# olegiy/manuscript-ocr

Hardware: AMD Instinct MI355X
Metric: manuscript pages/sec end-to-end (EAST+TRBA) at 1/2/4/8 MI355X; CER vs CPU ref (higher is better)
Workload: dtype f32 (bf16x3 split operands on the 1x1 / Winograd-domain GEMMs, f32 accumulate)

## Files before the change

include/msocr.h:

```cpp
#ifndef MSOCR_H
#define MSOCR_H
#include <stdint.h>

#ifdef __cplusplus
extern "C" {
#endif

#define MSOCR_F32 0
#define MSOCR_BF16 1

#define MSOCR_OK 0
#define MSOCR_E_ARG (-1)
#define MSOCR_E_LAUNCH (-2)
#define MSOCR_E_NOGPU (-3)

#define MSOCR_CONV_RELU 1u
#define MSOCR_CONV_RESIDUAL 2u
#define MSOCR_CONV_POOL2 4u

typedef struct msocr_conv_desc {
  int32_t dtype;
  int32_t N, H, W, Cin;
  int64_t in_sN, in_sH, in_sW;
  int32_t KH, KW, stride_h, stride_w, pad_h, pad_w;
  int32_t Ho, Wo, Cout;
  int64_t out_ld;
  int64_t res_ld;
  uint32_t flags;
} msocr_conv_desc;

int msocr_conv2d(const msocr_conv_desc* d, const void* in, const void* weight, const float* bias,
                 const void* residual, void* out, void* stream);

#define MSOCR_WINO_2X2 0
#define MSOCR_WINO_4X2 1
#define MSOCR_WINO_4X4 2
int64_t msocr_winograd_workspace_bytes(const msocr_conv_desc* d, int form);
int msocr_winograd_weights_host(int form, const float* w_khwc_host, int Cout, int Cin, float* u_out_host);
int msocr_conv3x3_winograd(const msocr_conv_desc* d, int form, int split, const void* in, const void* u, const float* bias,
                           const void* residual, void* out, void* workspace, void* stream);
int msocr_winograd_input_transform(const msocr_conv_desc* d, int form, const void* in, void* workspace, void* stream);
int msocr_winograd_gemm(const msocr_conv_desc* d, int form, int split, const void* u, void* workspace, void* stream);
int msocr_winograd_output_transform(const msocr_conv_desc* d, int form, const void* workspace, const float* bias, const void* residual,
                                    void* out, void* stream);

int msocr_split_bf16x3_host(const float* w_host, int64_t n, uint16_t* planes_out_host);
int msocr_split_bf16x3_ktile_host(const float* w_host, int64_t nbatch, int64_t rows, int64_t k, uint16_t* planes_out_host);
int msocr_conv1x1_split(const msocr_conv_desc* d, const void* in, const void* weight_planes, const float* bias,
                        const void* residual, void* out, void* stream);
int msocr_conv2d_split(const msocr_conv_desc* d, const void* in, const void* weight_planes, const float* bias,
                       const void* residual, void* out, void* stream);

int64_t msocr_winograd_fused64_workspace_bytes(const msocr_conv_desc* d);
int msocr_conv3x3_winograd_fused64(const msocr_conv_desc* d, int split, const void* in, const void* u, const float* bias,
                                   const void* residual, void* out, void* workspace, void* stream);
int msocr_winograd_fused64_gemm_output(const msocr_conv_desc* d, int split, const void* u, const void* workspace, const float* bias,
                                       const void* residual, void* out, void* stream);

int msocr_normalize_u8(const uint8_t* src, int N, int H, int W, int pad_t, int pad_l, int Hp, int Wp, int cpad,
                       int mode, int dtype, void* out, void* stream);

int msocr_resize_linear_u8(const uint8_t* src, int N, int sh, int sw, uint8_t* dst, int dh, int dw, void* stream);

int msocr_maxpool2d(const void* in, int N, int H, int W, int C, int64_t in_ld, int k, int s, int p, int dtype,
                    void* out, int Ho, int Wo, int64_t out_ld, void* stream);

int msocr_upsample2x_bilinear(const void* in, int N, int H, int W, int C, int64_t in_ld, int dtype, void* out,
                              int64_t out_ld, void* stream);

int msocr_east_head(const void* h1, int64_t npix, int64_t in_ld, int dtype, const float* w9, const float* b9,
                    float* score_out, float* geo_out, void* stream);

int msocr_east_decode(const float* score, const float* geo, int N, int H, int W, float thresh, float scale,
                      int quant, float* cand_out, int32_t* count_out, int max_cand, void* stream);

int64_t msocr_lanms_workspace_bytes(int N, int max_cand);
int msocr_east_lanms(const float* cand, const int32_t* counts, int N, int max_cand, double iou_thr, float* boxes_out,
                     int32_t* nbox_out, void* workspace, void* stream);

int64_t msocr_east_box_tail_workspace_bytes(int N, int max_cand);
int msocr_east_box_tail(const float* boxes, const int32_t* nbox, int N, int max_cand, double expand_w, double expand_h,
                        double scale_x, double scale_y, int axis_aligned_output, int remove_anomalies, double sigma, int min_count,
                        float* out, int32_t* n_out, void* workspace, void* stream);
int msocr_east_box_tail_host(const float* quads_host, int M, double expand_w, double expand_h, double scale_x, double scale_y,
                             int axis_aligned_output, int remove_anomalies, double sigma, int min_count, float* out_host,
                             int32_t* n_out_host);


int msocr_se_residual(const void* x, const void* identity, int N, int HW, int C, int dtype, const float* w1,
                      const float* w2, float* gate_ws, void* out, void* stream);

int msocr_mean_over_h(const void* in, int N, int H, int W, int C, int dtype, float* out, void* stream);

int msocr_bilstm_recurrent(const float* xproj, const float* w_hh_t, int B, int T, int H, float* hcat_out,
                           void* stream);
int msocr_bilstm_recurrent_split(const float* xproj, const uint16_t* whh_planes, int B, int T, int H, float* hcat_out,
                                 void* stream);

typedef struct msocr_attn_weights {
  const float* h2h_wt;
  const float* h2h_b;
  const float* score_w;
  const float* wih_ctx_t;
  const float* wih_tok;
  const float* whh_t;
  const float* b_gates;
  const float* gen_wt;
  const float* gen_b;
} msocr_attn_weights;

int msocr_attn_greedy(const float* batch_H, const float* proj_H, const msocr_attn_weights* w, int B, int T, int H,
                      int V, int steps, int sos_id, int eos_id, int blank_id, float* logits_out, int32_t* ids_out,
                      void* stream);
int64_t msocr_attn_beam_workspace_bytes(int B, int steps, int beam, int V);
int msocr_attn_beam(const float* batch_H, const float* proj_H, const msocr_attn_weights* w, int B, int T, int H,
                    int V, int steps, int beam, const float* lp_dev, float temperature, int sos_id, int eos_id,
                    int blank_id, int32_t* fin_step_out, void* workspace, const int32_t* chunk_id_dev,
                    const int32_t* chunk_size_dev, int32_t* chunk_state_dev, void* stream);
typedef struct msocr_attn_split_weights {
  const uint16_t* h2h_p;
  const uint16_t* whh_p;
  const uint16_t* gen_p;
} msocr_attn_split_weights;

int msocr_attn_beam_hoisted(const float* batch_H, const float* proj_H, const float* ctx_gates, const msocr_attn_weights* w,
                            const msocr_attn_split_weights* ws, int B, int T, int H, int V, int steps, int beam, const float* lp_dev,
                            float temperature, int sos_id, int eos_id, int blank_id, int32_t* fin_step_out, void* workspace,
                            const int32_t* chunk_id_dev, const int32_t* chunk_size_dev, int32_t* chunk_state_dev, void* stream);
int msocr_attn_greedy_hoisted(const float* batch_H, const float* proj_H, const float* ctx_gates, const msocr_attn_weights* w,
                              const msocr_attn_split_weights* ws, int B, int T, int H, int V, int steps, int sos_id, int eos_id,
                              int blank_id, float* logits_out, int32_t* ids_out, void* stream);
int64_t msocr_attn_pack_split_elems(int N);
int msocr_attn_pack_split_host(const float* wt_host, int N, int gate_interleaved, uint16_t* out_host);
int msocr_attn_beam_finalize(const void* workspace, int B, int V, int steps, int beam, const int32_t* trun_dev,
                             float* logits_out, int32_t* ids_out, void* stream);

int msocr_seq_confidence(const float* logits, const int32_t* ids, const int32_t* trun_dev, int B, int V, int steps,
                         float* conf_out, void* stream);

int msocr_crop_resize_pad(const uint8_t* pages, int N, int H, int W, const int32_t* desc_dev,
                          const int32_t* desc_host, int M, int img_h, int img_w, uint8_t* canvases, void* stream);

int msocr_reading_order_host(const int32_t* boxes_host, int n, double y_tol_ratio, double x_gap_ratio,
                             int32_t* order_out_host);

int64_t msocr_reading_order_workspace_bytes(int N, int max_cand);
int msocr_reading_order_crops(const float* boxes, const int32_t* nbox, int N, int max_cand, int page_h, int page_w,
                              int min_text_size, int img_h, int img_w, double y_tol_ratio, double x_gap_ratio, int page_base,
                              int32_t* order_out, int32_t* keep_out, int32_t* desc_out, int32_t* ncrop_out, void* workspace,
                              void* stream);

typedef struct msocr_jpeg_info {
  int32_t width, height, ncomp;
  int32_t hs[3], vs[3];
  int32_t blocks_w[3], blocks_h[3];
  int32_t supported;
  int64_t coef_off[3];
  int64_t coef_total;
  uint16_t quant[3][64];
} msocr_jpeg_info;
int msocr_jpeg_parse_host(const uint8_t* data_host, int64_t len, msocr_jpeg_info* info_out);
int msocr_jpeg_entropy_decode_host(const uint8_t* data_host, int64_t len, const msocr_jpeg_info* info, int16_t* coef_out_host);
int64_t msocr_jpeg_scan_desc_bytes(void);
int64_t msocr_jpeg_scan_prepare_host(const uint8_t* data_host, int64_t len, const msocr_jpeg_info* info, int64_t bytes_base,
                                     void* desc_out, uint32_t* bounds_out, int64_t bounds_cap);
int msocr_jpeg_entropy_decode_device(const uint8_t* bytes_dev, const void* descs_dev, int32_t n_pages, int32_t max_intervals,
                                     const uint32_t* bounds_dev, const int64_t* page_base_dev, int16_t* coef_dev, int64_t coef_total,
                                     int32_t* status_dev, void* stream);
int msocr_jpeg_entropy_decode_intervals_host(const uint8_t* bytes_host, const void* descs_host, int32_t n_pages,
                                             const uint32_t* bounds_host, const int64_t* page_base_host, int16_t* coef_host,
                                             int64_t coef_total, int32_t* status_host);
int64_t msocr_jpeg_workspace_bytes(const msocr_jpeg_info* info);
int msocr_jpeg_reconstruct(const msocr_jpeg_info* info, const int16_t* coef_dev, void* workspace_dev, uint8_t* rgb_out_dev,
                           void* stream);
int msocr_jpeg_reconstruct_host(const msocr_jpeg_info* info, const int16_t* coef_host, uint8_t* rgb_out_host);

int msocr_nchw_f32_to_nhwc(const float* in, int N, int C, int H, int W, int dtype, void* out, int64_t out_ld,
                           void* stream);
int msocr_nhwc_to_nchw_f32(const void* in, int N, int C, int H, int W, int64_t in_ld, int dtype, float* out,
                           void* stream);

const char* msocr_version(void);

#ifdef __cplusplus
}
#endif
#endif
```

manuscript_ocr_amd/_native.py:

```python
import ctypes
import os

import torch

_HERE = os.path.dirname(os.path.abspath(__file__))
LIB_PATH = os.path.join(_HERE, "libmsocr.so")

F32, BF16 = 0, 1
CONV_RELU, CONV_RESIDUAL, CONV_POOL2 = 1, 2, 4
WINO_2X2, WINO_4X2, WINO_4X4 = 0, 1, 2

c_i32, c_i64, c_u32 = ctypes.c_int32, ctypes.c_int64, ctypes.c_uint32
c_f32, c_f64, c_vp = ctypes.c_float, ctypes.c_double, ctypes.c_void_p


class ConvDesc(ctypes.Structure):
    _fields_ = [
        ("dtype", c_i32), ("N", c_i32), ("H", c_i32), ("W", c_i32), ("Cin", c_i32),
        ("in_sN", c_i64), ("in_sH", c_i64), ("in_sW", c_i64),
        ("KH", c_i32), ("KW", c_i32), ("stride_h", c_i32), ("stride_w", c_i32), ("pad_h", c_i32), ("pad_w", c_i32),
        ("Ho", c_i32), ("Wo", c_i32), ("Cout", c_i32),
        ("out_ld", c_i64), ("res_ld", c_i64), ("flags", c_u32),
    ]


class JpegInfo(ctypes.Structure):
    _fields_ = [("width", c_i32), ("height", c_i32), ("ncomp", c_i32), ("hs", c_i32 * 3), ("vs", c_i32 * 3),
                ("blocks_w", c_i32 * 3), ("blocks_h", c_i32 * 3), ("supported", c_i32), ("coef_off", c_i64 * 3),
                ("coef_total", c_i64), ("quant", (ctypes.c_uint16 * 64) * 3)]


class AttnWeights(ctypes.Structure):
    _fields_ = [(n, c_vp) for n in ("h2h_wt", "h2h_b", "score_w", "wih_ctx_t", "wih_tok", "whh_t", "b_gates", "gen_wt", "gen_b")]


class AttnSplitWeights(ctypes.Structure):
    _fields_ = [(n, c_vp) for n in ("h2h_p", "whh_p", "gen_p")]


_SIGS = {
    "msocr_conv2d": (c_i32, [ctypes.POINTER(ConvDesc), c_vp, c_vp, c_vp, c_vp, c_vp, c_vp]),
    "msocr_winograd_workspace_bytes": (c_i64, [ctypes.POINTER(ConvDesc), c_i32]),
    "msocr_winograd_weights_host": (c_i32, [c_i32, c_vp, c_i32, c_i32, c_vp]),
    "msocr_conv3x3_winograd": (c_i32, [ctypes.POINTER(ConvDesc), c_i32, c_i32, c_vp, c_vp, c_vp, c_vp, c_vp, c_vp, c_vp]),
    "msocr_winograd_input_transform": (c_i32, [ctypes.POINTER(ConvDesc), c_i32, c_vp, c_vp, c_vp]),
    "msocr_winograd_gemm": (c_i32, [ctypes.POINTER(ConvDesc), c_i32, c_i32, c_vp, c_vp, c_vp]),
    "msocr_winograd_output_transform": (c_i32, [ctypes.POINTER(ConvDesc), c_i32, c_vp, c_vp, c_vp, c_vp, c_vp]),
    "msocr_winograd_fused64_workspace_bytes": (c_i64, [ctypes.POINTER(ConvDesc)]),
    "msocr_conv3x3_winograd_fused64": (c_i32, [ctypes.POINTER(ConvDesc), c_i32, c_vp, c_vp, c_vp, c_vp, c_vp, c_vp, c_vp]),
    "msocr_winograd_fused64_gemm_output": (c_i32, [ctypes.POINTER(ConvDesc), c_i32, c_vp, c_vp, c_vp, c_vp, c_vp, c_vp]),
    "msocr_split_bf16x3_host": (c_i32, [c_vp, c_i64, c_vp]),
    "msocr_split_bf16x3_ktile_host": (c_i32, [c_vp, c_i64, c_i64, c_i64, c_vp]),
    "msocr_conv1x1_split": (c_i32, [ctypes.POINTER(ConvDesc), c_vp, c_vp, c_vp, c_vp, c_vp, c_vp]),
    "msocr_conv2d_split": (c_i32, [ctypes.POINTER(ConvDesc), c_vp, c_vp, c_vp, c_vp, c_vp, c_vp]),
    "msocr_normalize_u8": (c_i32, [c_vp, c_i32, c_i32, c_i32, c_i32, c_i32, c_i32, c_i32, c_i32, c_i32, c_i32, c_vp, c_vp]),
    "msocr_resize_linear_u8": (c_i32, [c_vp, c_i32, c_i32, c_i32, c_vp, c_i32, c_i32, c_vp]),
    "msocr_maxpool2d": (c_i32, [c_vp, c_i32, c_i32, c_i32, c_i32, c_i64, c_i32, c_i32, c_i32, c_i32, c_vp, c_i32, c_i32, c_i64, c_vp]),
    "msocr_upsample2x_bilinear": (c_i32, [c_vp, c_i32, c_i32, c_i32, c_i32, c_i64, c_i32, c_vp, c_i64, c_vp]),
    "msocr_east_head": (c_i32, [c_vp, c_i64, c_i64, c_i32, c_vp, c_vp, c_vp, c_vp, c_vp]),
    "msocr_east_decode": (c_i32, [c_vp, c_vp, c_i32, c_i32, c_i32, c_f32, c_f32, c_i32, c_vp, c_vp, c_i32, c_vp]),
    "msocr_lanms_workspace_bytes": (c_i64, [c_i32, c_i32]),
    "msocr_east_lanms": (c_i32, [c_vp, c_vp, c_i32, c_i32, c_f64, c_vp, c_vp, c_vp, c_vp]),
    "msocr_se_residual": (c_i32, [c_vp, c_vp, c_i32, c_i32, c_i32, c_i32, c_vp, c_vp, c_vp, c_vp, c_vp]),
    "msocr_mean_over_h": (c_i32, [c_vp, c_i32, c_i32, c_i32, c_i32, c_i32, c_vp, c_vp]),
    "msocr_bilstm_recurrent": (c_i32, [c_vp, c_vp, c_i32, c_i32, c_i32, c_vp, c_vp]),
    "msocr_bilstm_recurrent_split": (c_i32, [c_vp, c_vp, c_i32, c_i32, c_i32, c_vp, c_vp]),
    "msocr_attn_greedy": (c_i32, [c_vp, c_vp, ctypes.POINTER(AttnWeights), c_i32, c_i32, c_i32, c_i32, c_i32, c_i32, c_i32, c_i32,
                                  c_vp, c_vp, c_vp]),
    "msocr_attn_greedy_hoisted": (c_i32, [c_vp, c_vp, c_vp, ctypes.POINTER(AttnWeights), ctypes.POINTER(AttnSplitWeights), c_i32, c_i32,
                                          c_i32, c_i32, c_i32, c_i32, c_i32, c_i32, c_vp, c_vp, c_vp]),
    "msocr_attn_beam": (c_i32, [c_vp, c_vp, ctypes.POINTER(AttnWeights), c_i32, c_i32, c_i32, c_i32, c_i32, c_i32, c_vp, c_f32,
                                c_i32, c_i32, c_i32, c_vp, c_vp, c_vp, c_vp, c_vp, c_vp]),
    "msocr_attn_pack_split_elems": (c_i64, [c_i32]),
    "msocr_attn_pack_split_host": (c_i32, [c_vp, c_i32, c_i32, c_vp]),
    "msocr_attn_beam_hoisted": (c_i32, [c_vp, c_vp, c_vp, ctypes.POINTER(AttnWeights), ctypes.POINTER(AttnSplitWeights), c_i32, c_i32, c_i32, c_i32, c_i32, c_i32, c_vp, c_f32,
                                        c_i32, c_i32, c_i32, c_vp, c_vp, c_vp, c_vp, c_vp, c_vp]),
    "msocr_attn_beam_workspace_bytes": (c_i64, [c_i32, c_i32, c_i32, c_i32]),
    "msocr_attn_beam_finalize": (c_i32, [c_vp, c_i32, c_i32, c_i32, c_i32, c_vp, c_vp, c_vp, c_vp]),
    "msocr_seq_confidence": (c_i32, [c_vp, c_vp, c_vp, c_i32, c_i32, c_i32, c_vp, c_vp]),
    "msocr_crop_resize_pad": (c_i32, [c_vp, c_i32, c_i32, c_i32, c_vp, c_vp, c_i32, c_i32, c_i32, c_vp, c_vp]),
    "msocr_east_box_tail_workspace_bytes": (c_i64, [c_i32, c_i32]),
    "msocr_east_box_tail": (c_i32, [c_vp, c_vp, c_i32, c_i32, c_f64, c_f64, c_f64, c_f64, c_i32, c_i32, c_f64, c_i32, c_vp, c_vp, c_vp, c_vp]),
    "msocr_east_box_tail_host": (c_i32, [c_vp, c_i32, c_f64, c_f64, c_f64, c_f64, c_i32, c_i32, c_f64, c_i32, c_vp, c_vp]),
    "msocr_reading_order_host": (c_i32, [c_vp, c_i32, c_f64, c_f64, c_vp]),
    "msocr_reading_order_workspace_bytes": (c_i64, [c_i32, c_i32]),
    "msocr_reading_order_crops": (c_i32, [c_vp, c_vp, c_i32, c_i32, c_i32, c_i32, c_i32, c_i32, c_i32, c_f64, c_f64, c_i32,
                                          c_vp, c_vp, c_vp, c_vp, c_vp, c_vp]),
    "msocr_jpeg_parse_host": (c_i32, [c_vp, c_i64, ctypes.POINTER(JpegInfo)]),
    "msocr_jpeg_entropy_decode_host": (c_i32, [c_vp, c_i64, ctypes.POINTER(JpegInfo), c_vp]),
    "msocr_jpeg_scan_desc_bytes": (c_i64, []),
    "msocr_jpeg_scan_prepare_host": (c_i64, [c_vp, c_i64, ctypes.POINTER(JpegInfo), c_i64, c_vp, c_vp, c_i64]),
    "msocr_jpeg_entropy_decode_device": (c_i32, [c_vp, c_vp, c_i32, c_i32, c_vp, c_vp, c_vp, c_i64, c_vp, c_vp]),
    "msocr_jpeg_entropy_decode_intervals_host": (c_i32, [c_vp, c_vp, c_i32, c_vp, c_vp, c_vp, c_i64, c_vp]),
    "msocr_jpeg_workspace_bytes": (c_i64, [ctypes.POINTER(JpegInfo)]),
    "msocr_jpeg_reconstruct": (c_i32, [ctypes.POINTER(JpegInfo), c_vp, c_vp, c_vp, c_vp]),
    "msocr_jpeg_reconstruct_host": (c_i32, [ctypes.POINTER(JpegInfo), c_vp, c_vp]),
    "msocr_nchw_f32_to_nhwc": (c_i32, [c_vp, c_i32, c_i32, c_i32, c_i32, c_i32, c_vp, c_i64, c_vp]),
    "msocr_nhwc_to_nchw_f32": (c_i32, [c_vp, c_i32, c_i32, c_i32, c_i32, c_i64, c_i32, c_vp, c_vp]),
    "msocr_version": (ctypes.c_char_p, []),
}

_lib = None


class NativeError(RuntimeError):
    pass


def lib():
    global _lib
    if _lib is None:
        if not os.path.exists(LIB_PATH) and os.path.exists("/opt/rocm/bin/hipcc"):
            import fcntl
            import subprocess
            try:
                with open(os.path.join(_HERE, "csrc", ".build.lock"), "w") as lock:
                    fcntl.flock(lock, fcntl.LOCK_EX)
                    if not os.path.exists(LIB_PATH):
                        subprocess.check_call(["make", "-s", "-j4", "-C", os.path.join(_HERE, "csrc"), "ARCH=gfx950"])
            except Exception as e:
                print(f"[manuscript_ocr_amd] building libmsocr.so failed: {e}")
        if not os.path.exists(LIB_PATH):
            raise NativeError(
                f"{LIB_PATH} not found: build it with `python -c 'import __graft_entry__ as g; g.build()'` "
                "(or `make -C manuscript_ocr_amd/csrc`). There is no CPU fallback."
            )
        L = ctypes.CDLL(LIB_PATH)
        missing = [name for name in _SIGS if not hasattr(L, name)]
        if missing:
            raise NativeError(f"{LIB_PATH} lacks symbols declared in include/msocr.h: {missing}")
        for name, (res, args) in _SIGS.items():
            fn = getattr(L, name)
            fn.restype, fn.argtypes = res, args
        _lib = L
    return _lib


def exported_symbols():
    return list(_SIGS)


def check(rc, what):
    if rc != 0:
        raise NativeError(f"{what} failed with code {rc} (-1 bad argument/shape, -2 launch failure)")
```

manuscript_ocr_amd/csrc/trba_kernels.hip:

```cpp
#include <hip/hip_runtime.h>
#include <math.h>
#include <stdint.h>

#include "internal.h"
#include "msocr.h"

#define MSOCR_LAUNCH(...) do { (void)hipGetLastError(); hipLaunchKernelGGL(__VA_ARGS__); } while (0)
#define LAUNCH_OK() (hipGetLastError() == hipSuccess ? MSOCR_OK : MSOCR_E_LAUNCH)

typedef float f32x4 __attribute__((ext_vector_type(4)));

__device__ __forceinline__ float bf2f(uint16_t v) { return __uint_as_float(((uint32_t)v) << 16); }
__device__ __forceinline__ uint16_t f2bf(float f) {
  __bf16 b = (__bf16)f;
  return *reinterpret_cast<uint16_t*>(&b);
}
template <typename T> __device__ __forceinline__ float ldf(const T* p);
template <> __device__ __forceinline__ float ldf<float>(const float* p) { return *p; }
template <> __device__ __forceinline__ float ldf<uint16_t>(const uint16_t* p) { return bf2f(*p); }
template <typename T> __device__ __forceinline__ void stf(T* p, float v);
template <> __device__ __forceinline__ void stf<float>(float* p, float v) { *p = v; }
template <> __device__ __forceinline__ void stf<uint16_t>(uint16_t* p, float v) { *p = f2bf(v); }

__device__ __forceinline__ float sigmoidf_(float x) { return 1.0f / (1.0f + expf(-x)); }

__device__ __forceinline__ float wave_sum(float v) {
#pragma unroll
  for (int o = 32; o > 0; o >>= 1) v += __shfl_xor(v, o);
  return v;
}

template <typename T>
__device__ __forceinline__ f32x4 ld4(const T* p);
template <>
__device__ __forceinline__ f32x4 ld4<float>(const float* p) { return *reinterpret_cast<const f32x4*>(p); }
template <>
__device__ __forceinline__ f32x4 ld4<uint16_t>(const uint16_t* p) {
  const uint2 v = *reinterpret_cast<const uint2*>(p);
  f32x4 r = {bf2f((uint16_t)(v.x & 0xffff)), bf2f((uint16_t)(v.x >> 16)), bf2f((uint16_t)(v.y & 0xffff)), bf2f((uint16_t)(v.y >> 16))};
  return r;
}
template <typename T>
__device__ __forceinline__ void st4(T* p, f32x4 v);
template <>
__device__ __forceinline__ void st4<float>(float* p, f32x4 v) { *reinterpret_cast<f32x4*>(p) = v; }
template <>
__device__ __forceinline__ void st4<uint16_t>(uint16_t* p, f32x4 v) {
  uint2 o;
  o.x = (uint32_t)f2bf(v[0]) | ((uint32_t)f2bf(v[1]) << 16);
  o.y = (uint32_t)f2bf(v[2]) | ((uint32_t)f2bf(v[3]) << 16);
  *reinterpret_cast<uint2*>(p) = o;
}

template <typename T, int NT>
__global__ __launch_bounds__(NT) void se_residual_kernel(const T* __restrict__ x, const T* __restrict__ idt, int HW, int C,
                                                           const float* __restrict__ w1, const float* __restrict__ w2,
                                                           float* __restrict__ gate_ws, T* __restrict__ out) {
  extern __shared__ __attribute__((aligned(16))) float sm[];
  const int n = blockIdx.x, tid = threadIdx.x;
  const int C4 = C / 4, PG = NT / C4;
  float* part = sm;
  float* mean = sm + PG * C;
  float* hid = mean + C;
  float* gate = hid + C / 16;
  const T* xs = x + (long)n * HW * C;
  const int cg = tid % C4, pg = tid / C4;
  {
    f32x4 s = {0.f, 0.f, 0.f, 0.f};
    int p = pg;
    for (; p + 3 * PG < HW; p += 4 * PG) {
      f32x4 v[4];
#pragma unroll
      for (int u = 0; u < 4; ++u) v[u] = ld4<T>(xs + (long)(p + u * PG) * C + cg * 4);
#pragma unroll
      for (int u = 0; u < 4; ++u) { s[0] += v[u][0]; s[1] += v[u][1]; s[2] += v[u][2]; s[3] += v[u][3]; }
    }
    for (; p < HW; p += PG) {
      const f32x4 v = ld4<T>(xs + (long)p * C + cg * 4);
      s[0] += v[0]; s[1] += v[1]; s[2] += v[2]; s[3] += v[3];
    }
    *reinterpret_cast<f32x4*>(&part[pg * C + cg * 4]) = s;
  }
  __syncthreads();
  const float inv = 1.0f / (float)HW;
  for (int c = tid; c < C; c += NT) {
    float s = 0.f;
    for (int g = 0; g < PG; ++g) s += part[g * C + c];
    mean[c] = s * inv;
  }
  __syncthreads();
  const int Cr = C / 16;
  {
    const int lane = tid & 63, wv = tid >> 6;
    for (int j = wv; j < Cr; j += NT / 64) {
      float a = 0.f;
      for (int c = lane; c < C; c += 64) a = fmaf(w1[(long)j * C + c], mean[c], a);
      a = wave_sum(a);
      if (lane == 0) hid[j] = fmaxf(a, 0.f);
    }
  }
  __syncthreads();
  for (int c = tid; c < C; c += NT) {
    float a = 0.f;
    for (int j = 0; j < Cr; ++j) a = fmaf(w2[(long)c * Cr + j], hid[j], a);
    const float g = sigmoidf_(a);
    gate[c] = g;
    gate_ws[(long)n * C + c] = g;
  }
  __syncthreads();
  const T* is = idt + (long)n * HW * C;
  T* os = out + (long)n * HW * C;
  const f32x4 g4 = *reinterpret_cast<const f32x4*>(&gate[cg * 4]);
  int p = pg;
  for (; p + 3 * PG < HW; p += 4 * PG) {
    f32x4 v[4], r[4];
#pragma unroll
    for (int u = 0; u < 4; ++u) {
      const long o = (long)(p + u * PG) * C + cg * 4;
      v[u] = ld4<T>(xs + o);
      r[u] = ld4<T>(is + o);
    }
#pragma unroll
    for (int u = 0; u < 4; ++u) {
      f32x4 y;
#pragma unroll
      for (int e = 0; e < 4; ++e) y[e] = fmaxf(v[u][e] * g4[e] + r[u][e], 0.f);
      st4<T>(os + (long)(p + u * PG) * C + cg * 4, y);
    }
  }
  for (; p < HW; p += PG) {
    const long o = (long)p * C + cg * 4;
    const f32x4 v = ld4<T>(xs + o), r = ld4<T>(is + o);
    f32x4 y;
#pragma unroll
    for (int e = 0; e < 4; ++e) y[e] = fmaxf(v[e] * g4[e] + r[e], 0.f);
    st4<T>(os + o, y);
  }
}

extern "C" int msocr_se_residual(const void* x, const void* identity, int N, int HW, int C, int dtype, const float* w1, const float* w2,
                                 float* gate_ws, void* out, void* stream) {
  if (!x || !identity || !w1 || !w2 || !gate_ws || !out || N <= 0 || HW <= 0 || C < 64 || C > 1024 || (C & (C - 1))) return MSOCR_E_ARG;
  hipStream_t s = (hipStream_t)stream;
  if (dtype == MSOCR_F32) {
    MSOCR_LAUNCH((se_residual_kernel<float, 1024>), dim3(N), dim3(1024), (size_t)((1024 / (C / 4)) * C + 2 * C + C / 16) * sizeof(float), s,
                 (const float*)x, (const float*)identity, HW, C, w1, w2, gate_ws, (float*)out);
  } else if (dtype == MSOCR_BF16) {
    MSOCR_LAUNCH((se_residual_kernel<uint16_t, 256>), dim3(N), dim3(256), (size_t)((1024 / C) * C + 2 * C + C / 16) * sizeof(float), s,
                 (const uint16_t*)x, (const uint16_t*)identity, HW, C, w1, w2, gate_ws, (uint16_t*)out);
  } else {
    return MSOCR_E_ARG;
  }
  return LAUNCH_OK();
}

template <typename T>
__global__ void mean_over_h_kernel(const T* __restrict__ in, int N, int H, int W, int C, float* __restrict__ out) {
  const long total = (long)N * W * C;
  for (long i = blockIdx.x * (long)blockDim.x + threadIdx.x; i < total; i += (long)gridDim.x * blockDim.x) {
    const int c = (int)(i % C);
    const long t = i / C;
    const int w = (int)(t % W);
    const int n = (int)(t / W);
    float s = 0.f;
    for (int h = 0; h < H; ++h) s += ldf<T>(in + (((long)n * H + h) * W + w) * C + c);
    out[i] = s / (float)H;
  }
}
extern "C" int msocr_mean_over_h(const void* in, int N, int H, int W, int C, int dtype, float* out, void* stream) {
  if (!in || !out || N <= 0 || H <= 0 || W <= 0 || C <= 0) return MSOCR_E_ARG;
  const long total = (long)N * W * C;
  long g = (total + 255) / 256;
  if (g > 2048) g = 2048;
  hipStream_t s = (hipStream_t)stream;
  if (dtype == MSOCR_F32)
    MSOCR_LAUNCH(mean_over_h_kernel<float>, dim3((unsigned)g), dim3(256), 0, s, (const float*)in, N, H, W, C, out);
  else if (dtype == MSOCR_BF16)
    MSOCR_LAUNCH(mean_over_h_kernel<uint16_t>, dim3((unsigned)g), dim3(256), 0, s, (const uint16_t*)in, N, H, W, C, out);
  else
    return MSOCR_E_ARG;
  return LAUNCH_OK();
}

#define LSTM_RB 4
template <int H>
__global__ __launch_bounds__(H) void bilstm_kernel(const float* __restrict__ xproj, const float* __restrict__ whh_t, int B, int T,
                                                    float* __restrict__ hcat) {
  constexpr int G = 4 * H, RB = LSTM_RB;
  __shared__ __attribute__((aligned(16))) float hs[2][H][RB];
  const int j = threadIdx.x, d = blockIdx.y;
  const int b0 = blockIdx.x * RB;
  const float* wt = whh_t + (long)d * H * G;
  float c[RB];
#pragma unroll
  for (int r = 0; r < RB; ++r) {
    c[r] = 0.f;
    hs[0][j][r] = 0.f;
  }
  __syncthreads();
  for (int s = 0; s < T; ++s) {
    const int t = d == 0 ? s : T - 1 - s;
    const int cur = s & 1;
    float acc[4][RB];
#pragma unroll
    for (int r = 0; r < RB; ++r) {
      const int b = b0 + r < B ? b0 + r : B - 1;
      const float* xp = xproj + (((long)b * T + t) * 2 + d) * G;
#pragma unroll
      for (int g = 0; g < 4; ++g) acc[g][r] = xp[g * H + j];
    }
#pragma unroll 1
    for (int k0 = 0; k0 < H; k0 += 8) {
      f32x4 wq[8];
#pragma unroll
      for (int u = 0; u < 8; ++u) wq[u] = *reinterpret_cast<const f32x4*>(&wt[((long)(k0 + u) * H + j) * 4]);
#pragma unroll
      for (int u = 0; u < 8; ++u) {
        float hv[RB];
#pragma unroll
        for (int r4 = 0; r4 < RB; r4 += 4) {
          const f32x4 hq = *reinterpret_cast<const f32x4*>(&hs[cur][k0 + u][r4]);
          hv[r4] = hq[0]; hv[r4 + 1] = hq[1]; hv[r4 + 2] = hq[2]; hv[r4 + 3] = hq[3];
        }
#pragma unroll
        for (int g = 0; g < 4; ++g) {
#pragma unroll
          for (int r = 0; r < RB; ++r) acc[g][r] = fmaf(wq[u][g], hv[r], acc[g][r]);
        }
      }
    }
#pragma unroll
    for (int r = 0; r < RB; ++r) {
      const float ig = sigmoidf_(acc[0][r]), fg = sigmoidf_(acc[1][r]), gg = tanhf(acc[2][r]), og = sigmoidf_(acc[3][r]);
      c[r] = fg * c[r] + ig * gg;
      const float h = og * tanhf(c[r]);
      hs[cur ^ 1][j][r] = h;
      if (b0 + r < B) hcat[((long)(b0 + r) * T + t) * (2 * H) + d * H + j] = h;
    }
    __syncthreads();
  }
}

extern "C" int msocr_bilstm_recurrent(const float* xproj, const float* w_hh_t, int B, int T, int H, float* hcat_out, void* stream) {
  if (!xproj || !w_hh_t || !hcat_out || B <= 0 || T <= 0) return MSOCR_E_ARG;
  const dim3 grid((B + LSTM_RB - 1) / LSTM_RB, 2);
  if (H == 256) MSOCR_LAUNCH(bilstm_kernel<256>, grid, dim3(256), 0, (hipStream_t)stream, xproj, w_hh_t, B, T, hcat_out);
  else if (H == 128) MSOCR_LAUNCH(bilstm_kernel<128>, grid, dim3(128), 0, (hipStream_t)stream, xproj, w_hh_t, B, T, hcat_out);
  else if (H == 512) MSOCR_LAUNCH(bilstm_kernel<512>, grid, dim3(512), 0, (hipStream_t)stream, xproj, w_hh_t, B, T, hcat_out);
  else if (H == 64) MSOCR_LAUNCH(bilstm_kernel<64>, grid, dim3(64), 0, (hipStream_t)stream, xproj, w_hh_t, B, T, hcat_out);
  else if (H == 192) MSOCR_LAUNCH(bilstm_kernel<192>, grid, dim3(192), 0, (hipStream_t)stream, xproj, w_hh_t, B, T, hcat_out);
  else if (H == 320) MSOCR_LAUNCH(bilstm_kernel<320>, grid, dim3(320), 0, (hipStream_t)stream, xproj, w_hh_t, B, T, hcat_out);
  else if (H == 384) MSOCR_LAUNCH(bilstm_kernel<384>, grid, dim3(384), 0, (hipStream_t)stream, xproj, w_hh_t, B, T, hcat_out);
  else if (H == 448) MSOCR_LAUNCH(bilstm_kernel<448>, grid, dim3(448), 0, (hipStream_t)stream, xproj, w_hh_t, B, T, hcat_out);
  else return MSOCR_E_ARG;
  return LAUNCH_OK();
}


__global__ void attn_beam_finalize_kernel(const float* __restrict__ ws_logits, const int32_t* __restrict__ back,
                                          const int32_t* __restrict__ tokv, const int32_t* __restrict__ best_at,
                                          const int32_t* __restrict__ trun, int V, int steps, int K, float* __restrict__ logits_out,
                                          int32_t* __restrict__ ids_out) {
  const int b = blockIdx.x, tid = threadIdx.x;
  __shared__ int path[64];
  const int tr = trun[b];
  if (tid == 0) {
    int cur = best_at[(long)b * steps + tr - 1];
    for (int t = tr - 1; t >= 0; --t) {
      const long o = ((long)b * steps + t) * K + cur;
      ids_out[(long)b * steps + t] = tokv[o];
      path[t] = back[o];
      cur = back[o];
    }
    for (int t = tr; t < steps; ++t) ids_out[(long)b * steps + t] = -1;
  }
  __syncthreads();
  for (int t = 0; t < tr; ++t)
    for (int v = tid; v < V; v += blockDim.x)
      logits_out[((long)b * steps + t) * V + v] = ws_logits[(((long)b * steps + t) * K + path[t]) * V + v];
}

static bool attn_mfma_shape(int T, int H, int V) { return H == 256 && V <= 256 && T <= 48; }
static int check_attn(const float* bh, const float* ph, const msocr_attn_weights* w, int B, int T, int H, int V, int steps) {
  if (!bh || !ph || !w || B <= 0 || T <= 0 || T > 64 || H < 64 || H > 512 || H % 64 || V <= 0 || V > 512 || steps <= 0 || steps > 64)
    return MSOCR_E_ARG;
  if (!w->h2h_wt || !w->h2h_b || !w->score_w || !w->wih_ctx_t || !w->wih_tok || !w->whh_t || !w->b_gates || !w->gen_wt || !w->gen_b)
    return MSOCR_E_ARG;
  return MSOCR_OK;
}

extern "C" int msocr_attn_greedy(const float* batch_H, const float* proj_H, const msocr_attn_weights* w, int B, int T, int H, int V,
                                 int steps, int sos_id, int eos_id, int blank_id, float* logits_out, int32_t* ids_out, void* stream) {
  if (check_attn(batch_H, proj_H, w, B, T, H, V, steps) || !logits_out || !ids_out) return MSOCR_E_ARG;
  if (sos_id < 0 || sos_id >= V) return MSOCR_E_ARG;
  AttnArgs a{};
  a.batch_H = batch_H; a.proj_H = proj_H; a.w = *w;
  a.B = B; a.T = T; a.V = V; a.steps = steps; a.K = 1;
  a.sos_id = sos_id; a.eos_id = eos_id; a.blank_id = blank_id; a.temperature = 1.0f;
  a.logits_out = logits_out; a.ids_out = ids_out;
  return msocr_internal_attn_general(a, H, false, (hipStream_t)stream);
}

extern "C" int msocr_attn_greedy_hoisted(const float* batch_H, const float* proj_H, const float* ctx_gates, const msocr_attn_weights* w,
                                         const msocr_attn_split_weights* ws, int B, int T, int H, int V, int steps, int sos_id, int eos_id,
                                         int blank_id, float* logits_out, int32_t* ids_out, void* stream) {
  if (check_attn(batch_H, proj_H, w, B, T, H, V, steps) || !logits_out || !ids_out) return MSOCR_E_ARG;
  if (sos_id < 0 || sos_id >= V || !attn_mfma_shape(T, H, V)) return MSOCR_E_ARG;
  if (!ctx_gates || ((uintptr_t)ctx_gates & 15)) return MSOCR_E_ARG;
  if (!ws || !ws->h2h_p || !ws->whh_p || !ws->gen_p || (((uintptr_t)ws->h2h_p | (uintptr_t)ws->whh_p | (uintptr_t)ws->gen_p) & 15))
    return MSOCR_E_ARG;
  AttnArgs a{};
  a.batch_H = batch_H; a.proj_H = proj_H; a.w = *w; a.ctx_gates = ctx_gates;
  a.h2h_p = ws->h2h_p; a.whh_p = ws->whh_p; a.gen_p = ws->gen_p;
  a.B = B; a.T = T; a.V = V; a.steps = steps; a.K = 1;
  a.sos_id = sos_id; a.eos_id = eos_id; a.blank_id = blank_id; a.temperature = 1.0f;
  a.logits_out = logits_out; a.ids_out = ids_out;
  return msocr_internal_attn_greedy_mfma(a, (hipStream_t)stream);
}

static inline int64_t beam_ws_logits(int B, int steps, int K, int V) { return (int64_t)B * steps * K * V * 4; }
extern "C" int64_t msocr_attn_beam_workspace_bytes(int B, int steps, int beam, int V) {
  if (B <= 0 || steps <= 0 || beam <= 0 || V <= 0) return 0;
  return beam_ws_logits(B, steps, beam, V) + (int64_t)B * steps * beam * 8 + (int64_t)B * steps * 4 + 256;
}

static int attn_beam_impl(const float* batch_H, const float* proj_H, const float* ctx_gates, const msocr_attn_weights* w,
                          const msocr_attn_split_weights* ws, int B, int T, int H, int V, int steps, int beam, const float* lp_dev, float temperature, int sos_id, int eos_id, int blank_id,
                          int32_t* fin_step_out, void* workspace, const int32_t* chunk_id_dev, const int32_t* chunk_size_dev,
                          int32_t* chunk_state_dev, void* stream) {
  if (check_attn(batch_H, proj_H, w, B, T, H, V, steps) || !fin_step_out || !workspace) return MSOCR_E_ARG;
  if (beam < 1 || beam > 16 || sos_id < 0 || sos_id >= V || ((uintptr_t)workspace & 15)) return MSOCR_E_ARG;
  if (ctx_gates && (!attn_mfma_shape(T, H, V) || beam > 8)) return MSOCR_E_ARG;
  AttnArgs a{};
  a.batch_H = batch_H; a.proj_H = proj_H; a.w = *w; a.ctx_gates = ctx_gates;
  if (ws) { a.h2h_p = ws->h2h_p; a.whh_p = ws->whh_p; a.gen_p = ws->gen_p; }
  a.B = B; a.T = T; a.V = V; a.steps = steps; a.K = beam;
  a.sos_id = sos_id; a.eos_id = eos_id; a.blank_id = blank_id; a.temperature = temperature; a.lp = lp_dev;
  char* p = (char*)workspace;
  a.logits_out = (float*)p; p += beam_ws_logits(B, steps, beam, V);
  a.back = (int32_t*)p; p += (int64_t)B * steps * beam * 4;
  a.tokv = (int32_t*)p; p += (int64_t)B * steps * beam * 4;
  a.best_at = (int32_t*)p;
  a.fin_step = fin_step_out;
  if (chunk_id_dev && chunk_size_dev && chunk_state_dev) { a.chunk_id = chunk_id_dev; a.chunk_size = chunk_size_dev; a.chunk_state = chunk_state_dev; }
  if (!ctx_gates) return msocr_internal_attn_general(a, H, true, (hipStream_t)stream);
  return msocr_internal_attn_beam_mfma(a, (hipStream_t)stream);
}

extern "C" int msocr_attn_beam(const float* batch_H, const float* proj_H, const msocr_attn_weights* w, int B, int T, int H, int V,
                               int steps, int beam, const float* lp_dev, float temperature, int sos_id, int eos_id, int blank_id,
                               int32_t* fin_step_out, void* workspace, const int32_t* chunk_id_dev, const int32_t* chunk_size_dev,
                               int32_t* chunk_state_dev, void* stream) {
  return attn_beam_impl(batch_H, proj_H, nullptr, w, nullptr, B, T, H, V, steps, beam, lp_dev, temperature, sos_id, eos_id, blank_id, fin_step_out,
                        workspace, chunk_id_dev, chunk_size_dev, chunk_state_dev, stream);
}

extern "C" int msocr_attn_beam_hoisted(const float* batch_H, const float* proj_H, const float* ctx_gates, const msocr_attn_weights* w,
                                       const msocr_attn_split_weights* ws, int B, int T, int H, int V, int steps, int beam,
                                       const float* lp_dev, float temperature, int sos_id, int eos_id, int blank_id, int32_t* fin_step_out,
                                       void* workspace, const int32_t* chunk_id_dev, const int32_t* chunk_size_dev,
                                       int32_t* chunk_state_dev, void* stream) {
  if (!ctx_gates || ((uintptr_t)ctx_gates & 15)) return MSOCR_E_ARG;
  if (ws && (!ws->h2h_p || !ws->whh_p || !ws->gen_p || (((uintptr_t)ws->h2h_p | (uintptr_t)ws->whh_p | (uintptr_t)ws->gen_p) & 15)))
    return MSOCR_E_ARG;
  return attn_beam_impl(batch_H, proj_H, ctx_gates, w, ws, B, T, H, V, steps, beam, lp_dev, temperature, sos_id, eos_id, blank_id,
                        fin_step_out, workspace, chunk_id_dev, chunk_size_dev, chunk_state_dev, stream);
}

extern "C" int msocr_attn_beam_finalize(const void* workspace, int B, int V, int steps, int beam, const int32_t* trun_dev,
                                        float* logits_out, int32_t* ids_out, void* stream) {
  if (!workspace || !trun_dev || !logits_out || !ids_out || B <= 0 || V <= 0 || steps <= 0 || steps > 64 || beam < 1 || beam > 16)
    return MSOCR_E_ARG;
  const char* p = (const char*)workspace;
  const float* wl = (const float*)p; p += beam_ws_logits(B, steps, beam, V);
  const int32_t* back = (const int32_t*)p; p += (int64_t)B * steps * beam * 4;
  const int32_t* tokv = (const int32_t*)p; p += (int64_t)B * steps * beam * 4;
  const int32_t* best_at = (const int32_t*)p;
  MSOCR_LAUNCH(attn_beam_finalize_kernel, dim3(B), dim3(256), 0, (hipStream_t)stream, wl, back, tokv, best_at, trun_dev, V, steps, beam,
               logits_out, ids_out);
  return LAUNCH_OK();
}

__global__ __launch_bounds__(64) void seq_confidence_kernel(const float* __restrict__ logits, const int32_t* __restrict__ ids,
                                                             const int32_t* __restrict__ trun, int V, int steps,
                                                             float* __restrict__ conf) {
  const int b = blockIdx.x, lane = threadIdx.x;
  const int tr = trun[b];
  float acc = 0.f;
  for (int t = 0; t < tr; ++t) {
    const float* x = logits + ((long)b * steps + t) * V;
    float m = -INFINITY;
    for (int v = lane; v < V; v += 64) m = fmaxf(m, x[v]);
#pragma unroll
    for (int o = 32; o > 0; o >>= 1) m = fmaxf(m, __shfl_xor(m, o));
    float s = 0.f;
    for (int v = lane; v < V; v += 64) s += expf(x[v] - m);
    s = wave_sum(s);
    const int id = ids[(long)b * steps + t];
    const float logp = (x[id] - m) - logf(s);
    acc += expf(logp);
  }
  if (lane == 0) conf[b] = tr > 0 ? acc / (float)tr : 0.f;
}

extern "C" int msocr_seq_confidence(const float* logits, const int32_t* ids, const int32_t* trun_dev, int B, int V, int steps,
                                    float* conf_out, void* stream) {
  if (!logits || !ids || !trun_dev || !conf_out || B <= 0 || V <= 0 || steps <= 0) return MSOCR_E_ARG;
  MSOCR_LAUNCH(seq_confidence_kernel, dim3(B), dim3(64), 0, (hipStream_t)stream, logits, ids, trun_dev, V, steps, conf_out);
  return LAUNCH_OK();
}
```

manuscript_ocr_amd/csrc/winograd.hip:

```cpp
#include <hip/hip_runtime.h>
#include <stdint.h>

#include "internal.h"
#include "msocr.h"

#define MSOCR_LAUNCH(...) do { (void)hipGetLastError(); hipLaunchKernelGGL(__VA_ARGS__); } while (0)

typedef float f32x4 __attribute__((ext_vector_type(4)));

template <int M> __device__ void wino_bt1(const f32x4 d[M + 2], f32x4 r[M + 2]);
template <int M> __device__ void wino_at1(const f32x4 m[M + 2], f32x4 y[M]);

template <> __device__ __forceinline__ void wino_bt1<2>(const f32x4 d[4], f32x4 r[4]) {
  r[0] = d[0] - d[2];
  r[1] = d[1] + d[2];
  r[2] = d[2] - d[1];
  r[3] = d[1] - d[3];
}
template <> __device__ __forceinline__ void wino_at1<2>(const f32x4 m[4], f32x4 y[2]) {
  y[0] = (m[0] + m[1]) + m[2];
  y[1] = (m[1] - m[2]) - m[3];
}

__device__ __forceinline__ void wino44_bt(const f32x4 d[6], f32x4 r[6]) {
  constexpr float k97_36 = 97.0f / 36.0f, k4_9 = 4.0f / 9.0f, k9_4 = 2.25f, k3_2 = 1.5f, k2_3 = 2.0f / 3.0f;
#pragma unroll
  for (int e = 0; e < 4; ++e) {
    r[0][e] = fmaf(-k97_36, d[2][e], d[0][e]) + d[4][e];
    r[5][e] = fmaf(-k97_36, d[3][e], d[1][e]) + d[5][e];
    const float e1 = fmaf(-k4_9, d[2][e], d[4][e]), o1 = fmaf(k3_2, d[3][e], -k2_3 * d[1][e]);
    const float e2 = fmaf(-k9_4, d[2][e], d[4][e]), o2 = fmaf(k2_3, d[3][e], -k3_2 * d[1][e]);
    r[1][e] = e1 + o1; r[2][e] = e1 - o1;
    r[3][e] = e2 + o2; r[4][e] = e2 - o2;
  }
}
__device__ __forceinline__ void wino44_at(const f32x4 m[6], f32x4 y[4]) {
  constexpr float k3_2 = 1.5f, k2_3 = 2.0f / 3.0f, k9_4 = 2.25f, k4_9 = 4.0f / 9.0f, k27_8 = 3.375f, k8_27 = 8.0f / 27.0f;
#pragma unroll
  for (int e = 0; e < 4; ++e) {
    const float p12 = m[1][e] + m[2][e], d12 = m[1][e] - m[2][e], p34 = m[3][e] + m[4][e], d34 = m[3][e] - m[4][e];
    y[0][e] = (m[0][e] + p12) + p34;
    y[1][e] = fmaf(k3_2, d12, k2_3 * d34);
    y[2][e] = fmaf(k9_4, p12, k4_9 * p34);
    y[3][e] = fmaf(k27_8, d12, k8_27 * d34) + m[5][e];
  }
}
template <> __device__ __forceinline__ void wino_bt1<4>(const f32x4 d[6], f32x4 r[6]) { wino44_bt(d, r); }
template <> __device__ __forceinline__ void wino_at1<4>(const f32x4 m[6], f32x4 y[4]) { wino44_at(m, y); }


struct WinoGeom {
  int N, H, W;
  int TH, TW;
  long Mt;
};

template <int MH, int MW>
__device__ __forceinline__ void wino_input_body(const float* in, long sN, long sH, long sW, int C, WinoGeom g, float* V) {
  constexpr int PH = MH + 2, PW = MW + 2;
  constexpr bool w_first = MH == 4;
  const int cch = C >> 2;
  const long gid = (long)blockIdx.x * 256 + threadIdx.x;
  const long t = gid / cch;
  const int c = (int)(gid - t * cch) << 2;
  if (t >= g.Mt) return;
  const int tw = (int)(t % g.TW);
  const long r = t / g.TW;
  const int th = (int)(r % g.TH);
  const int n = (int)(r / g.TH);
  const int h0 = MH * th - 1, w0 = MW * tw - 1;
  const float* base = in + (long)n * sN + c;
  f32x4 q[PH][PW];
#pragma unroll
  for (int i = 0; i < PH; ++i) {
    const int hi = h0 + i;
    const bool okh = (unsigned)hi < (unsigned)g.H;
    f32x4 d[PW];
#pragma unroll
    for (int j = 0; j < PW; ++j) {
      const int wi = w0 + j;
      const bool ok = okh && (unsigned)wi < (unsigned)g.W;
      const f32x4 v = *reinterpret_cast<const f32x4*>(ok ? base + (long)hi * sH + (long)wi * sW : base);
      d[j] = ok ? v : (f32x4){0.f, 0.f, 0.f, 0.f};
    }
    if constexpr (w_first) {
      wino_bt1<MW>(d, q[i]);
    } else {
#pragma unroll
      for (int j = 0; j < PW; ++j) q[i][j] = d[j];
    }
  }
  const long plane = g.Mt * (long)C;
  float* o = V + t * (long)C + c;
  if constexpr (w_first) {
#pragma unroll
    for (int j = 0; j < PW; ++j) {
      f32x4 col[PH], v[PH];
#pragma unroll
      for (int i = 0; i < PH; ++i) col[i] = q[i][j];
      wino_bt1<MH>(col, v);
#pragma unroll
      for (int i = 0; i < PH; ++i) *reinterpret_cast<f32x4*>(o + (i * PW + j) * plane) = v[i];
    }
  } else {
#pragma unroll
    for (int i = 0; i < PH; ++i) {
      f32x4 row[PW], v[PW];
#pragma unroll
      for (int j = 0; j < PW; ++j) {
        f32x4 col[PH], hv[PH];
#pragma unroll
        for (int k = 0; k < PH; ++k) col[k] = q[k][j];
        wino_bt1<MH>(col, hv);
        row[j] = hv[i];
      }
      wino_bt1<MW>(row, v);
#pragma unroll
      for (int j = 0; j < PW; ++j) *reinterpret_cast<f32x4*>(o + (i * PW + j) * plane) = v[j];
    }
  }
}

template <int MH, int MW>
__device__ __forceinline__ void wino_output_body(const float* Mw, int Cout, WinoGeom g, const float* bias, const float* res, long res_ld,
                                                 int relu, float* out, long out_ld) {
  constexpr int PH = MH + 2, PW = MW + 2;
  const int cch = Cout >> 2;
  const long gid = (long)blockIdx.x * 256 + threadIdx.x;
  const long t = gid / cch;
  const int c = (int)(gid - t * cch) << 2;
  if (t >= g.Mt) return;
  const int tw = (int)(t % g.TW);
  const long r = t / g.TW;
  const int th = (int)(r % g.TH);
  const int n = (int)(r / g.TH);
  const long plane = g.Mt * (long)Cout;
  const float* mp = Mw + t * (long)Cout + c;
  f32x4 mt[PH][PW];
  if constexpr (MH == 2) {
#pragma unroll
    for (int i = 0; i < PH; ++i)
#pragma unroll
      for (int j = 0; j < PW; ++j) mt[i][j] = *reinterpret_cast<const f32x4*>(mp + (i * PW + j) * plane);
  }
  f32x4 s[MH][PW];
#pragma unroll
  for (int j = 0; j < PW; ++j) {
    f32x4 m[PH], y[MH];
#pragma unroll
    for (int i = 0; i < PH; ++i) m[i] = MH == 2 ? mt[i][j] : *reinterpret_cast<const f32x4*>(mp + (i * PW + j) * plane);
    wino_at1<MH>(m, y);
#pragma unroll
    for (int a = 0; a < MH; ++a) s[a][j] = y[a];
  }
  f32x4 b = {0.f, 0.f, 0.f, 0.f};
  if (bias) b = *reinterpret_cast<const f32x4*>(bias + c);
#pragma unroll
  for (int a = 0; a < MH; ++a) {
    const int ho = MH * th + a;
    if (ho >= g.H) continue;
    f32x4 y[MW];
    wino_at1<MW>(s[a], y);
#pragma unroll
    for (int j = 0; j < MW; ++j) {
      const int wo = MW * tw + j;
      if (wo >= g.W) continue;
      const long pix = ((long)n * g.H + ho) * g.W + wo;
      f32x4 v = y[j] + b;
      if (res) v += *reinterpret_cast<const f32x4*>(res + pix * res_ld + c);
      if (relu) {
        v[0] = fmaxf(v[0], 0.f); v[1] = fmaxf(v[1], 0.f); v[2] = fmaxf(v[2], 0.f); v[3] = fmaxf(v[3], 0.f);
      }
      *reinterpret_cast<f32x4*>(out + pix * out_ld + c) = v;
    }
  }
}

#define WINO_TRANSFORM_KERNELS(PREFIX, MH, MW)                                                                                    \
  __global__ __launch_bounds__(256) void PREFIX##_input_kernel(const float* __restrict__ in, long sN, long sH, long sW, int C,   \
                                                               WinoGeom g, float* __restrict__ V) {                            \
    wino_input_body<MH, MW>(in, sN, sH, sW, C, g, V);                                                                            \
  }                                                                                                                              \
  __global__ __launch_bounds__(256) void PREFIX##_output_kernel(const float* __restrict__ Mw, int Cout, WinoGeom g,              \
                                                                const float* __restrict__ bias, const float* __restrict__ res,  \
                                                                long res_ld, int relu, float* __restrict__ out, long out_ld) {  \
    wino_output_body<MH, MW>(Mw, Cout, g, bias, res, res_ld, relu, out, out_ld);                                                 \
  }
WINO_TRANSFORM_KERNELS(wino, 2, 2)
WINO_TRANSFORM_KERNELS(wino42, 4, 2)
WINO_TRANSFORM_KERNELS(wino44, 4, 4)
#undef WINO_TRANSFORM_KERNELS

static const int kWinoTile[3][2] = {{2, 2}, {4, 2}, {4, 4}};

static int wino_points(int form) { return (kWinoTile[form][0] + 2) * (kWinoTile[form][1] + 2); }

static bool wino_geom(const msocr_conv_desc* d, int form, WinoGeom* g) {
  if (form < MSOCR_WINO_2X2 || form > MSOCR_WINO_4X4 || !d || d->dtype != MSOCR_F32) return false;
  if (d->KH != 3 || d->KW != 3 || d->stride_h != 1 || d->stride_w != 1 || d->pad_h != 1 || d->pad_w != 1) return false;
  if (d->N <= 0 || d->H <= 0 || d->W <= 0 || d->Ho != d->H || d->Wo != d->W) return false;
  if (d->Cin <= 0 || d->Cin % 16 || d->Cout <= 0 || d->Cout % 32) return false;
  if ((long)d->N * ((d->H + 1) / 2) * ((d->W + 1) / 2) > 0x7fffffffL) return false;
  const int mh = kWinoTile[form][0], mw = kWinoTile[form][1];
  g->N = d->N; g->H = d->H; g->W = d->W;
  g->TH = (d->H + mh - 1) / mh; g->TW = (d->W + mw - 1) / mw;
  g->Mt = (long)d->N * g->TH * g->TW;
  return wino_points(form) * g->Mt * (long)(d->Cin > d->Cout ? d->Cin : d->Cout) <= 0x3fffffffffffL;
}

static bool wino_strides_ok(const msocr_conv_desc* d) { return !(d->in_sN % 4 || d->in_sH % 4 || d->in_sW % 4); }

static int wino_check(const msocr_conv_desc* d, int form, WinoGeom* g) {
  if (!wino_geom(d, form, g) || !wino_strides_ok(d) || d->out_ld % 4 || d->out_ld < d->Cout) return MSOCR_E_ARG;
  return MSOCR_OK;
}

static bool wino_gemm_ok(int form, int split) {
  if (split != 0 && split != 1) return false;
  return form == MSOCR_WINO_4X2 || (form == MSOCR_WINO_2X2 && !split) || (form == MSOCR_WINO_4X4 && split);
}

extern "C" int64_t msocr_winograd_workspace_bytes(const msocr_conv_desc* d, int form) {
  WinoGeom g;
  if (!wino_geom(d, form, &g)) return -1;
  return wino_points(form) * g.Mt * ((int64_t)d->Cin + d->Cout) * (int64_t)sizeof(float);
}

static int wino_launch_input(const msocr_conv_desc* d, int form, const WinoGeom& g, const void* in, void* workspace, void* stream) {
  if (!in || !workspace || (((uintptr_t)in | (uintptr_t)workspace) & 15)) return MSOCR_E_ARG;
  const long nb_in = (g.Mt * (d->Cin / 4) + 255) / 256;
  if (nb_in > 0x7fffffffL) return MSOCR_E_ARG;
  const dim3 grid((unsigned)nb_in), blk(256);
  hipStream_t st = (hipStream_t)stream;
  const float* x = (const float*)in;
  float* V = (float*)workspace;
  if (form == MSOCR_WINO_2X2) MSOCR_LAUNCH(wino_input_kernel, grid, blk, 0, st, x, (long)d->in_sN, (long)d->in_sH, (long)d->in_sW, d->Cin, g, V);
  else if (form == MSOCR_WINO_4X2) MSOCR_LAUNCH(wino42_input_kernel, grid, blk, 0, st, x, (long)d->in_sN, (long)d->in_sH, (long)d->in_sW, d->Cin, g, V);
  else MSOCR_LAUNCH(wino44_input_kernel, grid, blk, 0, st, x, (long)d->in_sN, (long)d->in_sH, (long)d->in_sW, d->Cin, g, V);
  return hipGetLastError() == hipSuccess ? MSOCR_OK : MSOCR_E_LAUNCH;
}

extern "C" int msocr_winograd_input_transform(const msocr_conv_desc* d, int form, const void* in, void* workspace, void* stream) {
  WinoGeom g;
  if (wino_check(d, form, &g) != MSOCR_OK) return MSOCR_E_ARG;
  return wino_launch_input(d, form, g, in, workspace, stream);
}

extern "C" int msocr_winograd_gemm(const msocr_conv_desc* d, int form, int split, const void* u, void* workspace, void* stream) {
  WinoGeom g;
  if (!wino_gemm_ok(form, split) || wino_check(d, form, &g) != MSOCR_OK || !u || !workspace) return MSOCR_E_ARG;
  if (split && (d->Cin % 32 || d->Cout % 64)) return MSOCR_E_ARG;
  const int P = wino_points(form);
  float* V = (float*)workspace;
  float* Mw = V + P * g.Mt * (long)d->Cin;
  if (split) return msocr_internal_gemm_split_batched(V, (const uint16_t*)u, Mw, g.Mt, d->Cout, d->Cin, P, (hipStream_t)stream);
  return msocr_internal_gemm_f32_batched(V, (const float*)u, Mw, g.Mt, d->Cout, d->Cin, P, (hipStream_t)stream);
}

extern "C" int msocr_winograd_output_transform(const msocr_conv_desc* d, int form, const void* workspace, const float* bias,
                                               const void* residual, void* out, void* stream) {
  WinoGeom g;
  if (wino_check(d, form, &g) != MSOCR_OK || !out || !workspace) return MSOCR_E_ARG;
  if (((uintptr_t)out | (uintptr_t)workspace) & 15) return MSOCR_E_ARG;
  const bool has_res = (d->flags & MSOCR_CONV_RESIDUAL) != 0;
  if (has_res && (!residual || d->res_ld % 4 || d->res_ld < d->Cout || ((uintptr_t)residual & 15))) return MSOCR_E_ARG;
  if (bias && ((uintptr_t)bias & 15)) return MSOCR_E_ARG;
  const long nb_out = (g.Mt * (d->Cout / 4) + 255) / 256;
  if (nb_out > 0x7fffffffL) return MSOCR_E_ARG;
  const float* Mw = (const float*)workspace + wino_points(form) * g.Mt * (long)d->Cin;
  const float* rp = has_res ? (const float*)residual : nullptr;
  const int relu = (d->flags & MSOCR_CONV_RELU) ? 1 : 0;
  const dim3 grid((unsigned)nb_out), blk(256);
  hipStream_t st = (hipStream_t)stream;
  float* o = (float*)out;
  if (form == MSOCR_WINO_2X2) MSOCR_LAUNCH(wino_output_kernel, grid, blk, 0, st, Mw, d->Cout, g, bias, rp, (long)d->res_ld, relu, o, (long)d->out_ld);
  else if (form == MSOCR_WINO_4X2) MSOCR_LAUNCH(wino42_output_kernel, grid, blk, 0, st, Mw, d->Cout, g, bias, rp, (long)d->res_ld, relu, o, (long)d->out_ld);
  else MSOCR_LAUNCH(wino44_output_kernel, grid, blk, 0, st, Mw, d->Cout, g, bias, rp, (long)d->res_ld, relu, o, (long)d->out_ld);
  return hipGetLastError() == hipSuccess ? MSOCR_OK : MSOCR_E_LAUNCH;
}

extern "C" int msocr_conv3x3_winograd(const msocr_conv_desc* d, int form, int split, const void* in, const void* u, const float* bias,
                                      const void* residual, void* out, void* workspace, void* stream) {
  if (!u || !wino_gemm_ok(form, split)) return MSOCR_E_ARG;
  int rc = msocr_winograd_input_transform(d, form, in, workspace, stream);
  if (rc != MSOCR_OK) return rc;
  rc = msocr_winograd_gemm(d, form, split, u, workspace, stream);
  if (rc != MSOCR_OK) return rc;
  return msocr_winograd_output_transform(d, form, workspace, bias, residual, out, stream);
}

typedef unsigned int u32x4w __attribute__((ext_vector_type(4)));
#ifndef WINO_FUSED_PFD
#define WINO_FUSED_PFD 3
#endif

typedef __bf16 bf16x8w __attribute__((ext_vector_type(8)));
typedef unsigned int u32x2w __attribute__((ext_vector_type(2)));
__device__ __forceinline__ unsigned int wino_split_step(float& x, float& y) {
  typedef __bf16 bf16x2 __attribute__((ext_vector_type(2)));
  typedef float f32x2 __attribute__((ext_vector_type(2)));
  const f32x2 v = {x, y};
  const bf16x2 h = __builtin_convertvector(v, bf16x2);
  const unsigned int pk = __builtin_bit_cast(unsigned int, h);
  x -= __uint_as_float(pk << 16);
  y -= __uint_as_float(pk & 0xffff0000u);
  return pk;
}

template <bool POOL, bool SPLIT = false>
__global__ __launch_bounds__(256, 3) void wino42_fused64_kernel(const float* __restrict__ V, const void* __restrict__ Uv, int Cout,
                                                                 WinoGeom g, const float* __restrict__ bias,
                                                                 const float* __restrict__ res, long res_ld, int relu,
                                                                 float* __restrict__ out, long out_ld) {
  constexpr int K = 64, BM = 32, BN = 32, ROWB = K * 4;
  constexpr int ROWS = 128, PLANE = BM * ROWS;
  constexpr int STAGE_BYTES = SPLIT ? 6 * PLANE : (BM + BN) * ROWB;
  __shared__ __attribute__((aligned(16))) unsigned char smem[2][STAGE_BYTES];
  const int tid = threadIdx.x, lane = tid & 63, wave = tid >> 6;
  const int mi = wave >> 1, nj = wave & 1;
  const int r16 = lane & 15, kg = lane >> 4;
  const int nbn = Cout / BN;
  const long nblk = (long)gridDim.x;
  long bid = blockIdx.x;
  {
    const long q = nblk >> 3, r = nblk & 7, x = bid & 7;
    bid = (x < r ? x * (q + 1) : r * (q + 1) + (x - r) * q) + (bid >> 3);
  }
  const int nb = (int)(bid % nbn);
  const long m0 = (bid / nbn) * BM;
  const int n0 = nb * BN;
  f32x4 acc[24];

  if constexpr (SPLIT) {
    const unsigned short* U = reinterpret_cast<const unsigned short*>(Uv);
    const int chunk = tid & 15, row0 = tid >> 4;
    const int bchunk = tid & 7, brow = tid >> 3;
    const long planeV = g.Mt * (long)K, planeU = (long)Cout * K, uplane = 24 * planeU;
    const float* pa[2];
#pragma unroll
    for (int i = 0; i < 2; ++i) {
      long m = m0 + row0 + 16 * i;
      if (m >= g.Mt) m = g.Mt - 1;
      pa[i] = V + m * K + chunk * 4;
    }
    const unsigned short* pb = U + (long)(n0 + brow) * K + bchunk * 8;
    constexpr int PFD = 2;
    u32x4w ra[PFD][2], rb[PFD][3];
    auto gload = [&](int p) {
#pragma unroll
      for (int i = 0; i < 2; ++i) ra[p % PFD][i] = *reinterpret_cast<const u32x4w*>(pa[i] + p * planeV);
#pragma unroll
      for (int pl = 0; pl < 3; ++pl) rb[p % PFD][pl] = *reinterpret_cast<const u32x4w*>(pb + pl * uplane + p * planeU);
    };
    auto sstore = [&](int p) {
      unsigned char* st = &smem[p & 1][0];
#pragma unroll
      for (int i = 0; i < 2; ++i) {
        const int row = row0 + 16 * i;
        float x0 = __uint_as_float(ra[p % PFD][i][0]), x1 = __uint_as_float(ra[p % PFD][i][1]);
        float x2 = __uint_as_float(ra[p % PFD][i][2]), x3 = __uint_as_float(ra[p % PFD][i][3]);
        unsigned char* dst = st + row * ROWS + (((chunk >> 1) ^ (row & 7)) << 4) + ((chunk & 1) << 3);
#pragma unroll
        for (int pl = 0; pl < 3; ++pl) {
          u32x2w v;
          v[0] = wino_split_step(x0, x1);
          v[1] = wino_split_step(x2, x3);
          *reinterpret_cast<u32x2w*>(dst + pl * PLANE) = v;
        }
      }
#pragma unroll
      for (int pl = 0; pl < 3; ++pl)
        *reinterpret_cast<u32x4w*>(st + (3 + pl) * PLANE + brow * ROWS + ((bchunk ^ (brow & 7)) << 4)) = rb[p % PFD][pl];
    };
#pragma unroll
    for (int q = 0; q < PFD; ++q) gload(q);
    sstore(0);
    __syncthreads();
#pragma unroll
    for (int p = 0; p < 24; ++p) {
      if (p + PFD < 24) gload(p + PFD);
      const unsigned char* st = &smem[p & 1][0];
      const int rowa = mi * 16 + r16, rowb = nj * 16 + r16;
      f32x4 c4 = {0.f, 0.f, 0.f, 0.f};
#pragma unroll
      for (int ks = 0; ks < 2; ++ks) {
        const int c = 4 * ks + kg;
        bf16x8w fa[3], fb[3];
#pragma unroll
        for (int pl = 0; pl < 3; ++pl) {
          fa[pl] = *reinterpret_cast<const bf16x8w*>(st + pl * PLANE + rowa * ROWS + ((c ^ (rowa & 7)) << 4));
          fb[pl] = *reinterpret_cast<const bf16x8w*>(st + (3 + pl) * PLANE + rowb * ROWS + ((c ^ (rowb & 7)) << 4));
        }
        c4 = __builtin_amdgcn_mfma_f32_16x16x32_bf16(fa[2], fb[0], c4, 0, 0, 0);
        c4 = __builtin_amdgcn_mfma_f32_16x16x32_bf16(fa[0], fb[2], c4, 0, 0, 0);
        c4 = __builtin_amdgcn_mfma_f32_16x16x32_bf16(fa[1], fb[1], c4, 0, 0, 0);
        c4 = __builtin_amdgcn_mfma_f32_16x16x32_bf16(fa[1], fb[0], c4, 0, 0, 0);
        c4 = __builtin_amdgcn_mfma_f32_16x16x32_bf16(fa[0], fb[1], c4, 0, 0, 0);
        c4 = __builtin_amdgcn_mfma_f32_16x16x32_bf16(fa[0], fb[0], c4, 0, 0, 0);
      }
      acc[p] = c4;
      if (p + 1 < 24) sstore(p + 1);
      __syncthreads();
    }
  } else {
  const float* U = reinterpret_cast<const float*>(Uv);
  const int chunk = tid & 15, row0 = tid >> 4;
  const long planeV = g.Mt * (long)K, planeU = (long)Cout * K;
  const float* pa[2];
  const float* pb[2];
#pragma unroll
  for (int i = 0; i < 2; ++i) {
    long m = m0 + row0 + 16 * i;
    if (m >= g.Mt) m = g.Mt - 1;
    pa[i] = V + m * K + chunk * 4;
    pb[i] = U + (long)(n0 + row0 + 16 * i) * K + chunk * 4;
  }
  constexpr int PFD = WINO_FUSED_PFD;
  u32x4w ra[PFD][2], rb[PFD][2];
  auto gload = [&](int p) {
#pragma unroll
    for (int i = 0; i < 2; ++i) {
      ra[p % PFD][i] = *reinterpret_cast<const u32x4w*>(pa[i] + p * planeV);
      rb[p % PFD][i] = *reinterpret_cast<const u32x4w*>(pb[i] + p * planeU);
    }
  };
  auto sstore = [&](int p) {
#pragma unroll
    for (int i = 0; i < 2; ++i) {
      const int row = row0 + 16 * i;
      *reinterpret_cast<u32x4w*>(&smem[p & 1][row * ROWB + ((chunk ^ (row & 15)) << 4)]) = ra[p % PFD][i];
      *reinterpret_cast<u32x4w*>(&smem[p & 1][(BM + row) * ROWB + ((chunk ^ (row & 15)) << 4)]) = rb[p % PFD][i];
    }
  };
#pragma unroll
  for (int q = 0; q < PFD; ++q) gload(q);
  sstore(0);
  __syncthreads();
#pragma unroll
  for (int p = 0; p < 24; ++p) {
    if (p + PFD < 24) gload(p + PFD);
    const unsigned char* sa = &smem[p & 1][0];
    const unsigned char* sb = sa + BM * ROWB;
    const int rowa = mi * 16 + r16, rowb = nj * 16 + r16;
    u32x4w fa[4], fb[4];
#pragma unroll
    for (int q = 0; q < 4; ++q) {
      const int c = kg * 4 + q;
      fa[q] = *reinterpret_cast<const u32x4w*>(sa + rowa * ROWB + ((c ^ (rowa & 15)) << 4));
      fb[q] = *reinterpret_cast<const u32x4w*>(sb + rowb * ROWB + ((c ^ (rowb & 15)) << 4));
    }
    f32x4 c4 = {0.f, 0.f, 0.f, 0.f};
#pragma unroll
    for (int q = 0; q < 4; ++q)
#pragma unroll
      for (int e = 0; e < 4; ++e)
        c4 = __builtin_amdgcn_mfma_f32_16x16x4f32(__uint_as_float(fa[q][e]), __uint_as_float(fb[q][e]), c4, 0, 0, 0);
    acc[p] = c4;
    if (p + 1 < 24) sstore(p + 1);
    __syncthreads();
  }

  }

  const int co = n0 + nj * 16 + r16;
  const float b = bias ? bias[co] : 0.f;
#pragma unroll
  for (int e = 0; e < 4; ++e) {
    const long t = m0 + mi * 16 + 4 * kg + e;
    if (t >= g.Mt) continue;
    const int tw = (int)(t % g.TW);
    const long r = t / g.TW;
    const int th = (int)(r % g.TH);
    const int n = (int)(r / g.TH);
    float s[4][4];
#pragma unroll
    for (int j = 0; j < 4; ++j) {
      const float m0_ = acc[0 * 4 + j][e], m1 = acc[1 * 4 + j][e], m2 = acc[2 * 4 + j][e], m3 = acc[3 * 4 + j][e], m4 = acc[4 * 4 + j][e],
                  m5 = acc[5 * 4 + j][e];
      const float p12 = m1 + m2, d12 = m1 - m2, p34 = m3 + m4, d34 = m3 - m4;
      s[0][j] = (m0_ + p12) + p34;
      s[1][j] = fmaf(1.5f, d12, (2.0f / 3.0f) * d34);
      s[2][j] = fmaf(2.25f, p12, (4.0f / 9.0f) * p34);
      s[3][j] = fmaf(3.375f, d12, (8.0f / 27.0f) * d34) + m5;
    }
    float y[4][2];
#pragma unroll
    for (int i = 0; i < 4; ++i) {
      y[i][0] = ((s[i][0] + s[i][1]) + s[i][2]) + b;
      y[i][1] = ((s[i][1] - s[i][2]) - s[i][3]) + b;
    }
    if constexpr (POOL) {
      const int Hp = g.H >> 1, Wp = g.W >> 1;
#pragma unroll
      for (int i2 = 0; i2 < 2; ++i2) {
        const int hp = 2 * th + i2;
        if (hp >= Hp || tw >= Wp) continue;
        float v0 = y[2 * i2][0], v1 = y[2 * i2][1], v2 = y[2 * i2 + 1][0], v3 = y[2 * i2 + 1][1];
        if (relu) { v0 = fmaxf(v0, 0.f); v1 = fmaxf(v1, 0.f); v2 = fmaxf(v2, 0.f); v3 = fmaxf(v3, 0.f); }
        out[(((long)n * Hp + hp) * Wp + tw) * out_ld + co] = fmaxf(fmaxf(v0, v1), fmaxf(v2, v3));
      }
    } else {
#pragma unroll
      for (int i = 0; i < 4; ++i) {
        const int ho = 4 * th + i;
        if (ho >= g.H) continue;
#pragma unroll
        for (int j = 0; j < 2; ++j) {
          const int wo = 2 * tw + j;
          if (wo >= g.W) continue;
          const long pix = ((long)n * g.H + ho) * g.W + wo;
          float v = y[i][j];
          if (res) v += res[pix * res_ld + co];
          if (relu) v = fmaxf(v, 0.f);
          out[pix * out_ld + co] = v;
        }
      }
    }
  }
}

template <bool POOL>
__global__ __launch_bounds__(256, 2) void wino42_fused64_v2_kernel(const float* __restrict__ V, const unsigned short* __restrict__ U, int Cout,
                                                                    WinoGeom g, const float* __restrict__ bias,
                                                                    const float* __restrict__ res, long res_ld, int relu,
                                                                    float* __restrict__ out, long out_ld) {
  constexpr int K = 64, BM = 64, BN = 64, ROWS = 128, PLANE = BM * ROWS;
  typedef float f32x16w __attribute__((ext_vector_type(16)));
  __shared__ __attribute__((aligned(16))) unsigned char smem[6 * PLANE];
  const int tid = threadIdx.x, lane = tid & 63, wave = tid >> 6;
  const int wm = wave >> 1, wn = wave & 1;
  const int r32 = lane & 31, half = lane >> 5;
  const int nbn = Cout / BN;
  const long nblk = (long)gridDim.x;
  long bid = blockIdx.x;
  {
    const long q = nblk >> 3, r = nblk & 7, x = bid & 7;
    bid = (x < r ? x * (q + 1) : r * (q + 1) + (x - r) * q) + (bid >> 3);
  }
  const int nb = (int)(bid % nbn);
  const long m0 = (bid / nbn) * BM;
  const int n0 = nb * BN;

  const int chunk = tid & 15, row0 = tid >> 4;
  const int bchunk = tid & 7, brow = tid >> 3;
  const long planeV = g.Mt * (long)K, planeU = (long)Cout * K, uplane = 24 * planeU;
  const float* pa[4];
#pragma unroll
  for (int i = 0; i < 4; ++i) {
    long m = m0 + row0 + 16 * i;
    if (m >= g.Mt) m = g.Mt - 1;
    pa[i] = V + m * K + chunk * 4;
  }
  const unsigned short* pb = U + (long)(n0 + brow) * K + bchunk * 8;
  u32x4w ra[4], rb[3][2];
  auto gload = [&](int p) {
#pragma unroll
    for (int i = 0; i < 4; ++i) ra[i] = *reinterpret_cast<const u32x4w*>(pa[i] + p * planeV);
#pragma unroll
    for (int pl = 0; pl < 3; ++pl)
#pragma unroll
      for (int j = 0; j < 2; ++j) rb[pl][j] = *reinterpret_cast<const u32x4w*>(pb + pl * uplane + p * planeU + (long)j * 32 * K);
  };
  auto sstore = [&]() {
#pragma unroll
    for (int i = 0; i < 4; ++i) {
      const int row = row0 + 16 * i;
      float x0 = __uint_as_float(ra[i][0]), x1 = __uint_as_float(ra[i][1]), x2 = __uint_as_float(ra[i][2]), x3 = __uint_as_float(ra[i][3]);
      unsigned char* dst = smem + row * ROWS + (((chunk >> 1) ^ (row & 7)) << 4) + ((chunk & 1) << 3);
#pragma unroll
      for (int pl = 0; pl < 3; ++pl) {
        u32x2w v;
        v[0] = wino_split_step(x0, x1);
        v[1] = wino_split_step(x2, x3);
        *reinterpret_cast<u32x2w*>(dst + pl * PLANE) = v;
      }
    }
#pragma unroll
    for (int pl = 0; pl < 3; ++pl)
#pragma unroll
      for (int j = 0; j < 2; ++j) {
        const int row = brow + 32 * j;
        *reinterpret_cast<u32x4w*>(smem + (3 + pl) * PLANE + row * ROWS + ((bchunk ^ (row & 7)) << 4)) = rb[pl][j];
      }
  };

  f32x16w Y[8];
#pragma unroll
  for (int o = 0; o < 8; ++o)
#pragma unroll
    for (int e = 0; e < 16; ++e) Y[o][e] = 0.f;

  gload(0);
  sstore();
  __syncthreads();
  __shared__ float s_cf[24][8];
  if (tid < 192) {
    const float t6[4][6] = {{1, 1, 1, 1, 1, 0}, {0, 1.5f, -1.5f, 2.0f / 3.0f, -2.0f / 3.0f, 0}, {0, 2.25f, 2.25f, 4.0f / 9.0f, 4.0f / 9.0f, 0},
                            {0, 3.375f, -3.375f, 8.0f / 27.0f, -8.0f / 27.0f, 1}};
    const float t4[2][4] = {{1, 1, 1, 0}, {0, 1, -1, -1}};
    const int pp = tid >> 3, o = tid & 7;
    s_cf[pp][o] = t6[o >> 1][pp >> 2] * t4[o & 1][pp & 3];
  }
  __syncthreads();
  const int rowa = wm * 32 + r32, rowb = wn * 32 + r32;
#pragma unroll 1
  for (int p = 0; p < 24; ++p) {
    if (p + 1 < 24) gload(p + 1);
    f32x16w m;
#pragma unroll
    for (int e = 0; e < 16; ++e) m[e] = 0.f;
#pragma unroll
    for (int ks = 0; ks < 4; ++ks) {
      const int c = 2 * ks + half;
      bf16x8w fa[3], fb[3];
#pragma unroll
      for (int pl = 0; pl < 3; ++pl) {
        fa[pl] = *reinterpret_cast<const bf16x8w*>(smem + pl * PLANE + rowa * ROWS + ((c ^ (rowa & 7)) << 4));
        fb[pl] = *reinterpret_cast<const bf16x8w*>(smem + (3 + pl) * PLANE + rowb * ROWS + ((c ^ (rowb & 7)) << 4));
      }
      m = __builtin_amdgcn_mfma_f32_32x32x16_bf16(fa[2], fb[0], m, 0, 0, 0);
      m = __builtin_amdgcn_mfma_f32_32x32x16_bf16(fa[0], fb[2], m, 0, 0, 0);
      m = __builtin_amdgcn_mfma_f32_32x32x16_bf16(fa[1], fb[1], m, 0, 0, 0);
      m = __builtin_amdgcn_mfma_f32_32x32x16_bf16(fa[1], fb[0], m, 0, 0, 0);
      m = __builtin_amdgcn_mfma_f32_32x32x16_bf16(fa[0], fb[1], m, 0, 0, 0);
      m = __builtin_amdgcn_mfma_f32_32x32x16_bf16(fa[0], fb[0], m, 0, 0, 0);
    }
#pragma unroll
    for (int o = 0; o < 8; ++o) {
      const float cf = s_cf[p][o];
#pragma unroll
      for (int e = 0; e < 16; ++e) Y[o][e] = fmaf(cf, m[e], Y[o][e]);
    }
    __syncthreads();
    if (p + 1 < 24) sstore();
    __syncthreads();
  }

  const int co = n0 + wn * 32 + r32;
  const float bv = bias ? bias[co] : 0.f;
#pragma unroll
  for (int e = 0; e < 16; ++e) {
    const long t = m0 + wm * 32 + (e & 3) + 8 * (e >> 2) + 4 * half;
    if (t >= g.Mt) continue;
    const int tw = (int)(t % g.TW);
    const long r = t / g.TW;
    const int th = (int)(r % g.TH);
    const int n = (int)(r / g.TH);
    if constexpr (POOL) {
      const int Hp = g.H >> 1, Wp = g.W >> 1;
#pragma unroll
      for (int i2 = 0; i2 < 2; ++i2) {
        const int hp = 2 * th + i2;
        if (hp >= Hp || tw >= Wp) continue;
        float v0 = Y[4 * i2 + 0][e] + bv, v1 = Y[4 * i2 + 1][e] + bv, v2 = Y[4 * i2 + 2][e] + bv, v3 = Y[4 * i2 + 3][e] + bv;
        if (relu) { v0 = fmaxf(v0, 0.f); v1 = fmaxf(v1, 0.f); v2 = fmaxf(v2, 0.f); v3 = fmaxf(v3, 0.f); }
        out[(((long)n * Hp + hp) * Wp + tw) * out_ld + co] = fmaxf(fmaxf(v0, v1), fmaxf(v2, v3));
      }
    } else {
#pragma unroll
      for (int a = 0; a < 4; ++a) {
        const int ho = 4 * th + a;
        if (ho >= g.H) continue;
#pragma unroll
        for (int b = 0; b < 2; ++b) {
          const int wo = 2 * tw + b;
          if (wo >= g.W) continue;
          const long pix = ((long)n * g.H + ho) * g.W + wo;
          float v = Y[a * 2 + b][e] + bv;
          if (res) v += res[pix * res_ld + co];
          if (relu) v = fmaxf(v, 0.f);
          out[pix * out_ld + co] = v;
        }
      }
    }
  }
}

static int wino_fused64_check(const msocr_conv_desc* d, WinoGeom* g) {
  if (!wino_geom(d, MSOCR_WINO_4X2, g) || d->Cin != 64 || !wino_strides_ok(d) || d->out_ld < d->Cout) return MSOCR_E_ARG;
  if (d->flags & MSOCR_CONV_POOL2) {
    if ((d->H & 1) || (d->W & 1) || (d->flags & MSOCR_CONV_RESIDUAL)) return MSOCR_E_ARG;
  }
  return MSOCR_OK;
}

extern "C" int64_t msocr_winograd_fused64_workspace_bytes(const msocr_conv_desc* d) {
  WinoGeom g;
  if (wino_fused64_check(d, &g) != MSOCR_OK) return -1;
  return 24 * g.Mt * (int64_t)d->Cin * (int64_t)sizeof(float);
}

extern "C" int msocr_winograd_fused64_gemm_output(const msocr_conv_desc* d, int split, const void* u, const void* workspace,
                                                  const float* bias, const void* residual, void* out, void* stream) {
  WinoGeom g;
  if ((split != 0 && split != 1) || wino_fused64_check(d, &g) != MSOCR_OK || !u || !workspace || !out) return MSOCR_E_ARG;
  if (((uintptr_t)workspace | (uintptr_t)u) & 15) return MSOCR_E_ARG;
  const bool has_res = (d->flags & MSOCR_CONV_RESIDUAL) != 0;
  if (has_res && (!residual || d->res_ld < d->Cout)) return MSOCR_E_ARG;
  const long nblk = ((g.Mt + 31) / 32) * (long)(d->Cout / 32);
  if (nblk <= 0 || nblk > 0x7fffffffL) return MSOCR_E_ARG;
  const int relu = (d->flags & MSOCR_CONV_RELU) ? 1 : 0;
  const float* rp = has_res ? (const float*)residual : nullptr;
  const dim3 grid((unsigned)nblk), blk(256);
  hipStream_t st = (hipStream_t)stream;
  const float* ws = (const float*)workspace;
  if (split && d->Cout % 64 == 0) {
    const long nblk2 = ((g.Mt + 63) / 64) * (long)(d->Cout / 64);
    if (nblk2 <= 0 || nblk2 > 0x7fffffffL) return MSOCR_E_ARG;
    const dim3 grid2((unsigned)nblk2);
    const unsigned short* up = (const unsigned short*)u;
    if (d->flags & MSOCR_CONV_POOL2)
      MSOCR_LAUNCH((wino42_fused64_v2_kernel<true>), grid2, blk, 0, st, ws, up, d->Cout, g, bias, (const float*)nullptr, 0L, relu, (float*)out, (long)d->out_ld);
    else
      MSOCR_LAUNCH((wino42_fused64_v2_kernel<false>), grid2, blk, 0, st, ws, up, d->Cout, g, bias, rp, (long)d->res_ld, relu, (float*)out, (long)d->out_ld);
    return hipGetLastError() == hipSuccess ? MSOCR_OK : MSOCR_E_LAUNCH;
  }
  if (d->flags & MSOCR_CONV_POOL2) {
    if (split) MSOCR_LAUNCH((wino42_fused64_kernel<true, true>), grid, blk, 0, st, ws, u, d->Cout, g, bias, (const float*)nullptr, 0L, relu, (float*)out, (long)d->out_ld);
    else MSOCR_LAUNCH((wino42_fused64_kernel<true, false>), grid, blk, 0, st, ws, u, d->Cout, g, bias, (const float*)nullptr, 0L, relu, (float*)out, (long)d->out_ld);
  } else {
    if (split) MSOCR_LAUNCH((wino42_fused64_kernel<false, true>), grid, blk, 0, st, ws, u, d->Cout, g, bias, rp, (long)d->res_ld, relu, (float*)out, (long)d->out_ld);
    else MSOCR_LAUNCH((wino42_fused64_kernel<false, false>), grid, blk, 0, st, ws, u, d->Cout, g, bias, rp, (long)d->res_ld, relu, (float*)out, (long)d->out_ld);
  }
  return hipGetLastError() == hipSuccess ? MSOCR_OK : MSOCR_E_LAUNCH;
}

extern "C" int msocr_conv3x3_winograd_fused64(const msocr_conv_desc* d, int split, const void* in, const void* u, const float* bias,
                                              const void* residual, void* out, void* workspace, void* stream) {
  WinoGeom g;
  if ((split != 0 && split != 1) || wino_fused64_check(d, &g) != MSOCR_OK || !u) return MSOCR_E_ARG;
  const int rc = wino_launch_input(d, MSOCR_WINO_4X2, g, in, workspace, stream);
  if (rc != MSOCR_OK) return rc;
  return msocr_winograd_fused64_gemm_output(d, split, u, workspace, bias, residual, out, stream);
}

extern "C" int msocr_winograd_weights_host(int form, const float* w_khwc, int Cout, int Cin, float* u_out) {
  if (form < MSOCR_WINO_2X2 || form > MSOCR_WINO_4X4 || !w_khwc || !u_out || Cout <= 0 || Cin <= 0) return MSOCR_E_ARG;
  static const double G4[4][3] = {{1.0, 0.0, 0.0}, {0.5, 0.5, 0.5}, {0.5, -0.5, 0.5}, {0.0, 0.0, 1.0}};
  static const double G6[6][3] = {{1.0, 0.0, 0.0},
                                  {8.0 / 65, 12.0 / 65, 18.0 / 65},     {8.0 / 65, -12.0 / 65, 18.0 / 65},
                                  {-81.0 / 130, -27.0 / 65, -18.0 / 65}, {-81.0 / 130, 27.0 / 65, -18.0 / 65},
                                  {0.0, 0.0, 1.0}};
  const int PH = kWinoTile[form][0] + 2, PW = kWinoTile[form][1] + 2;
  const double(*Gh)[3] = PH == 6 ? G6 : G4;
  const double(*Gw)[3] = PW == 6 ? G6 : G4;
  const long plane = (long)Cout * Cin;
  for (int co = 0; co < Cout; ++co) {
    const float* w = w_khwc + (long)co * 9 * Cin;
    for (int c = 0; c < Cin; ++c) {
      double gw[6][3];
      for (int xi = 0; xi < PH; ++xi)
        for (int kw = 0; kw < 3; ++kw)
          gw[xi][kw] = Gh[xi][0] * w[(0 * 3 + kw) * Cin + c] + Gh[xi][1] * w[(1 * 3 + kw) * Cin + c] + Gh[xi][2] * w[(2 * 3 + kw) * Cin + c];
      for (int xi = 0; xi < PH; ++xi)
        for (int nu = 0; nu < PW; ++nu)
          u_out[(xi * PW + nu) * plane + (long)co * Cin + c] =
              (float)(gw[xi][0] * Gw[nu][0] + gw[xi][1] * Gw[nu][1] + gw[xi][2] * Gw[nu][2]);
    }
  }
  return MSOCR_OK;
}
```

manuscript_ocr_amd/ops.py:

```python
import ctypes
import os

import torch

from . import _native as nat


PROFILE = None


def _prof_begin():
    if PROFILE is None:
        return None
    e0 = torch.cuda.Event(enable_timing=True)
    e0.record()
    return e0


def _prof_end(e0, kind, work, tag=None):
    if e0 is None or PROFILE is None:
        return
    e1 = torch.cuda.Event(enable_timing=True)
    e1.record()
    PROFILE.append((e0, e1, kind, work, tag))


def _dt(t):
    if t.dtype == torch.float32:
        return nat.F32
    if t.dtype == torch.bfloat16:
        return nat.BF16
    raise TypeError(f"unsupported dtype {t.dtype}")


def _stream():
    return ctypes.c_void_p(torch.cuda.current_stream().cuda_stream)


def _need_cuda(*ts):
    for t in ts:
        if t is not None and not t.is_cuda:
            raise nat.NativeError("native ops need device tensors (no CPU fallback)")


def _pixel_dense_ld(t):
    N, H, W, C = t.shape
    ld = t.stride(2)
    if t.stride(3) != 1 or t.stride(1) != W * ld or (N > 1 and t.stride(0) != H * W * ld) or ld < C:
        raise ValueError(f"tensor is not pixel-dense NHWC: shape {tuple(t.shape)} strides {t.stride()}")
    return ld


WINOGRAD_MIN_CIN = int(os.environ.get("MSOCR_WINOGRAD_MIN_CIN", "128"))


WINO_WS_LIMIT = int(os.environ.get("MSOCR_WINO_WS_LIMIT", str(1 << 30)))
_WINO_ARENA = {}


def _wino_workspace(nbytes, device):
    if torch.cuda.is_current_stream_capturing():
        return torch.empty((nbytes,), dtype=torch.uint8, device=device)
    key = (device.index, torch.cuda.current_stream().cuda_stream)
    buf = _WINO_ARENA.get(key)
    if buf is None or buf.numel() < nbytes:
        buf = None
        _WINO_ARENA.pop(key, None)
        buf = torch.empty((nbytes,), dtype=torch.uint8, device=device)
        _WINO_ARENA[key] = buf
    return buf


WINOGRAD_TALL = int(os.environ.get("MSOCR_WINO_TALL", "1"))


def _tall_pays(H):
    return 24 * (-(-H // 4)) < 16 * (-(-H // 2))


WINOGRAD_SQUARE = int(os.environ.get("MSOCR_WINO_SQUARE", "1"))
WINOGRAD_SQUARE_MIN_CIN = int(os.environ.get("MSOCR_WINO_SQUARE_MIN_CIN", "512"))


def _square_pays(W):
    return 36 * (-(-W // 4)) < 24 * (-(-W // 2))


WINO_FORMS = {nat.WINO_2X2: ("winograd", 16, (2, 2)), nat.WINO_4X2: ("winograd42", 24, (4, 2)), nat.WINO_4X4: ("winograd44", 36, (4, 4))}


def _wino_weights(wh, form):
    Cout, _, _, Cin = wh.shape
    u = torch.empty((WINO_FORMS[form][1], Cout, Cin), dtype=torch.float32)
    nat.check(nat.lib().msocr_winograd_weights_host(form, wh.data_ptr(), Cout, Cin, u.data_ptr()), "winograd_weights_host")
    return u


WINOGRAD_FUSED64 = int(os.environ.get("MSOCR_WINO_FUSED64", "1"))


SPLIT_BF16X3 = int(os.environ.get("MSOCR_SPLIT", "1"))


def split_planes(t):
    th = t.detach().float().cpu().contiguous()
    planes = torch.empty((3,) + tuple(th.shape), dtype=torch.int16)
    nat.check(nat.lib().msocr_split_bf16x3_host(th.data_ptr(), th.numel(), planes.data_ptr()), "split_bf16x3_host")
    return planes.view(torch.bfloat16).to(t.device)


def split_planes_ktile(t, nbatch, rows):
    th = t.detach().float().cpu().contiguous()
    k = th.numel() // (nbatch * rows)
    assert k % 32 == 0 and nbatch * rows * k == th.numel()
    planes = torch.empty((3, nbatch, k // 32, rows, 32), dtype=torch.int16)
    nat.check(nat.lib().msocr_split_bf16x3_ktile_host(th.data_ptr(), nbatch, rows, k, planes.data_ptr()), "split_bf16x3_ktile_host")
    return planes.view(torch.bfloat16).to(t.device)


def unsplit_planes_ktile(planes):
    nb, kt, rows = planes.shape[1:4]
    return planes.float().sum(0).permute(0, 2, 1, 3).reshape(nb, rows, kt * 32)


SPLIT_MIN_K = int(os.environ.get("MSOCR_SPLIT_MIN_K", "128"))


def _split_eligible(w):
    Cout, KH, KW, Cin = w.shape
    return w.dtype == torch.float32 and Cin % 32 == 0 and Cout % 64 == 0 and KH * KW * Cin >= SPLIT_MIN_K


def attach_split(w, split=None):
    if split is False:
        w._msocr_nosplit = True
        return w
    Cout, KH, KW, Cin = w.shape
    if (SPLIT_BF16X3 if split is None else split) and KH == 1 and KW == 1 and _split_eligible(w):
        w._msocr_split = split_planes_ktile(w, 1, Cout)
    return w


def attach_winograd(w, split=None, square=True):
    Cout, KH, KW, Cin = w.shape
    if (WINOGRAD_MIN_CIN and WINOGRAD_FUSED64 and WINOGRAD_TALL and w.dtype == torch.float32 and KH == 3 and KW == 3 and Cin == 64
            and Cin < WINOGRAD_MIN_CIN and Cout % 32 == 0):
        u42 = _wino_weights(w.detach().cpu().contiguous(), nat.WINO_4X2)
        w._msocr_wino42_fused = u42.to(w.device)
        if (SPLIT_BF16X3 if split is None else split) and (Cout % 64 == 0 or Cout >= 128):
            w._msocr_wino42_fused_split = split_planes(u42).to(w.device)
        return w
    if not (WINOGRAD_MIN_CIN and w.dtype == torch.float32 and KH == 3 and KW == 3 and Cin >= WINOGRAD_MIN_CIN and Cin % 16 == 0
            and Cout % 32 == 0):
        return w
    wh = w.detach().cpu().contiguous()
    w._msocr_wino = _wino_weights(wh, nat.WINO_2X2).to(w.device)
    u42 = _wino_weights(wh, nat.WINO_4X2)
    w._msocr_wino42 = u42.to(w.device)
    if (SPLIT_BF16X3 if split is None else split) and Cin % 32 == 0 and Cout % 64 == 0:
        w._msocr_wino42_split = split_planes_ktile(u42, 24, Cout).to(w.device)
        if WINOGRAD_SQUARE and square and Cin >= WINOGRAD_SQUARE_MIN_CIN:
            w._msocr_wino44_split = split_planes_ktile(_wino_weights(wh, nat.WINO_4X4), 36, Cout).to(w.device)
    return w


def _winograd(d, x, w, u, form, split, bias, residual, out, alg, fused=False, pool2=False):
    N, H, W, Cin = x.shape
    Cout = w.shape[0]
    stem, npts, (mh, mw) = WINO_FORMS[form]
    name = stem + ("_fused" if fused else "") + ("_split" if split else "")
    L = nat.lib()
    nbytes = L.msocr_winograd_fused64_workspace_bytes(ctypes.byref(d)) if fused else L.msocr_winograd_workspace_bytes(ctypes.byref(d), form)
    if nbytes < 0:
        raise nat.NativeError(f"{name}: unsupported shape {tuple(x.shape)} * {tuple(w.shape)} pool2={pool2}")
    parts = min(N, -(-nbytes // WINO_WS_LIMIT))
    per = -(-N // parts)
    ws = _wino_workspace(nbytes if parts == 1 else (nbytes // N) * per, x.device)
    bp = bias.data_ptr() if bias is not None else None
    what = f"msocr_conv3x3_{name} {tuple(x.shape)} * {tuple(w.shape)}"
    TH, TW = -(-H // mh), -(-W // mw)
    out_px = H * W // (4 if pool2 else 1)
    res_io = 2 if residual is not None else 1
    for n0 in range(0, N, per):
        n1 = min(N, n0 + per)
        d.N = n1 - n0
        xp, rp, op = x[n0:n1].data_ptr(), (residual[n0:n1].data_ptr() if residual is not None else None), out[n0:n1].data_ptr()
        if PROFILE is None:
            if fused:
                rc = L.msocr_conv3x3_winograd_fused64(ctypes.byref(d), int(split), xp, u.data_ptr(), bp, rp, op, ws.data_ptr(), _stream())
            else:
                rc = L.msocr_conv3x3_winograd(ctypes.byref(d), form, int(split), xp, u.data_ptr(), bp, rp, op, ws.data_ptr(), _stream())
            nat.check(rc, what)
            continue
        nn, mt = n1 - n0, (n1 - n0) * TH * TW
        e = _prof_begin()
        nat.check(L.msocr_winograd_input_transform(ctypes.byref(d), form, xp, ws.data_ptr(), _stream()), what)
        _prof_end(e, "wino_in", 4.0 * (nn * H * W * Cin + npts * mt * Cin), (mt, Cin))
        e = _prof_begin()
        if fused:
            rc = L.msocr_winograd_fused64_gemm_output(ctypes.byref(d), int(split), u.data_ptr(), ws.data_ptr(), bp, rp, op, _stream())
        else:
            rc = L.msocr_winograd_gemm(ctypes.byref(d), form, int(split), u.data_ptr(), ws.data_ptr(), _stream())
        nat.check(rc, what)
        io = x.element_size() * (nn * H * W * Cin + nn * out_px * Cout * res_io + Cout * 9 * Cin)
        _prof_end(e, "conv_gemm", (alg * nn / N, 2.0 * npts * mt * Cin * Cout, io), (nn * H * W, Cout, 9 * Cin, name))
        if not fused:
            e = _prof_begin()
            nat.check(L.msocr_winograd_output_transform(ctypes.byref(d), form, ws.data_ptr(), bp, rp, op, _stream()), what)
            _prof_end(e, "wino_out", 4.0 * (npts * mt * Cout + nn * H * W * Cout * res_io), (mt, Cout))
    d.N = N


def conv2d(x, w, bias, stride=(1, 1), pad=(0, 0), relu=False, residual=None, out=None, out_hw=None, alg_k=None, pool2=False):
    _need_cuda(x, w, bias, residual, out)
    N, H, W, Cin = x.shape
    Cout, KH, KW, Cw = w.shape
    assert Cw == Cin and w.is_contiguous() and w.dtype == x.dtype and x.stride(3) == 1
    sh, sw = stride
    ph, pw = pad
    Ho, Wo = out_hw if out_hw else ((H + 2 * ph - KH) // sh + 1, (W + 2 * pw - KW) // sw + 1)
    wino = (sh, sw, ph, pw) == (1, 1, 1, 1) and (Ho, Wo) == (H, W)
    fused = (getattr(w, "_msocr_wino42_fused", None) is not None and WINOGRAD_FUSED64 and WINOGRAD_TALL and wino and _tall_pays(H)
             and (not pool2 or (H % 2 == 0 and W % 2 == 0 and residual is None)))
    if pool2 and not fused:
        return maxpool2d(conv2d(x, w, bias, stride, pad, relu, residual, None, out_hw, alg_k), 2, 2, 0, out=out)
    u = getattr(w, "_msocr_wino", None)
    use_wino = u is not None and wino
    oh, ow = (Ho // 2, Wo // 2) if pool2 else (Ho, Wo)
    if out is None:
        out = torch.empty((N, oh, ow, Cout), dtype=x.dtype, device=x.device)
    assert out.shape == (N, oh, ow, Cout) and out.dtype == x.dtype
    d = nat.ConvDesc()
    d.dtype = _dt(x)
    d.N, d.H, d.W, d.Cin = N, H, W, Cin
    d.in_sN, d.in_sH, d.in_sW = x.stride(0), x.stride(1), x.stride(2)
    d.KH, d.KW, d.stride_h, d.stride_w, d.pad_h, d.pad_w = KH, KW, sh, sw, ph, pw
    d.Ho, d.Wo, d.Cout = Ho, Wo, Cout
    d.out_ld = _pixel_dense_ld(out)
    flags = (nat.CONV_RELU if relu else 0) | (nat.CONV_POOL2 if pool2 else 0)
    rp = None
    if residual is not None:
        assert residual.shape == out.shape and residual.dtype == x.dtype
        d.res_ld = _pixel_dense_ld(residual)
        flags |= nat.CONV_RESIDUAL
        rp = residual.data_ptr()
    d.flags = flags
    if bias is not None:
        assert bias.dtype == torch.float32 and bias.numel() == Cout and bias.is_contiguous()
    bp = bias.data_ptr() if bias is not None else None
    alg = 2.0 * N * Ho * Wo * Cout * (alg_k if alg_k else KH * KW * Cin)
    if fused:
        up = getattr(w, "_msocr_wino42_fused_split", None) if SPLIT_BF16X3 else None
        u = w._msocr_wino42_fused if up is None else up
        _winograd(d, x, w, u, nat.WINO_4X2, up is not None, bias, residual, out, alg, fused=True, pool2=pool2)
    elif use_wino:
        form, split = nat.WINO_2X2, False
        if WINOGRAD_TALL and _tall_pays(H) and getattr(w, "_msocr_wino42", None) is not None:
            form, u = nat.WINO_4X2, w._msocr_wino42
            up = getattr(w, "_msocr_wino42_split", None)
            if up is not None and SPLIT_BF16X3:
                u, split = up, True
            up44 = getattr(w, "_msocr_wino44_split", None)
            if up44 is not None and SPLIT_BF16X3 and WINOGRAD_SQUARE and _square_pays(W):
                form, u, split = nat.WINO_4X4, up44, True
        _winograd(d, x, w, u, form, split, bias, residual, out, alg)
    else:
        wp = getattr(w, "_msocr_split", None)
        if (wp is None and SPLIT_BF16X3 and not getattr(w, "_msocr_nosplit", False) and _split_eligible(w)
                and not torch.cuda.is_current_stream_capturing()):
            wp = w._msocr_split = split_planes_ktile(w, 1, Cout)
        split = wp is not None and SPLIT_BF16X3 and KH * KW * Cin >= SPLIT_MIN_K and all(v % 4 == 0 for v in x.stride()[:3])
        lean = (split and (KH, KW, sh, sw, ph, pw) == (1, 1, 1, 1, 0, 0) and (Ho, Wo) == (H, W)
                and (H == 1 or x.stride(1) == W * x.stride(2)) and (N == 1 or x.stride(0) == H * W * x.stride(2)))
        e = _prof_begin()
        if split:
            fn = nat.lib().msocr_conv1x1_split if lean else nat.lib().msocr_conv2d_split
            rc = fn(ctypes.byref(d), x.data_ptr(), wp.data_ptr(), bp, rp, out.data_ptr(), _stream())
            nat.check(rc, f"msocr_conv{'1x1' if lean else '2d'}_split {tuple(x.shape)} * {tuple(w.shape)}")
        else:
            rc = nat.lib().msocr_conv2d(ctypes.byref(d), x.data_ptr(), w.data_ptr(), bp, rp, out.data_ptr(), _stream())
            nat.check(rc, f"msocr_conv2d {tuple(x.shape)} * {tuple(w.shape)}")
        io = x.element_size() * (N * H * W * Cin + N * Ho * Wo * Cout * (2 if residual is not None else 1) + Cout * KH * KW * Cin)
        _prof_end(e, "conv_gemm", (alg, 2.0 * N * Ho * Wo * Cout * KH * KW * Cin, io),
                  (N * Ho * Wo, Cout, KH * KW * Cin, "direct_split" if split else "direct"))
    return out


def normalize_u8(imgs_u8, pad_t, pad_l, Hp, Wp, mode, dtype, cpad=4):
    _need_cuda(imgs_u8)
    N, H, W, C = imgs_u8.shape
    assert C == 3 and imgs_u8.dtype == torch.uint8 and imgs_u8.is_contiguous()
    out = torch.empty((N, Hp, Wp, cpad), dtype=dtype, device=imgs_u8.device)
    nat.check(nat.lib().msocr_normalize_u8(imgs_u8.data_ptr(), N, H, W, pad_t, pad_l, Hp, Wp, cpad, mode, _dt(out), out.data_ptr(),
                                           _stream()),
              "normalize_u8")
    return out


def resize_linear_u8(src, dh, dw):
    _need_cuda(src)
    N, sh, sw, C = src.shape
    assert C == 3 and src.dtype == torch.uint8 and src.is_contiguous()
    dst = torch.empty((N, dh, dw, 3), dtype=torch.uint8, device=src.device)
    nat.check(nat.lib().msocr_resize_linear_u8(src.data_ptr(), N, sh, sw, dst.data_ptr(), dh, dw, _stream()), "resize_linear_u8")
    return dst


def maxpool2d(x, k, s, p, out=None):
    _need_cuda(x, out)
    N, H, W, C = x.shape
    Ho, Wo = (H + 2 * p - k) // s + 1, (W + 2 * p - k) // s + 1
    if out is None:
        out = torch.empty((N, Ho, Wo, C), dtype=x.dtype, device=x.device)
    e = _prof_begin()
    nat.check(nat.lib().msocr_maxpool2d(x.data_ptr(), N, H, W, C, _pixel_dense_ld(x), k, s, p, _dt(x), out.data_ptr(), Ho, Wo,
                                        _pixel_dense_ld(out), _stream()), "maxpool2d")
    _prof_end(e, "maxpool", float(x.element_size()) * N * C * (H * W + Ho * Wo))
    return out


def upsample2x_into(x, out):
    _need_cuda(x, out)
    N, H, W, C = x.shape
    assert out.shape[0] == N and out.shape[1] == 2 * H and out.shape[2] == 2 * W and out.dtype == x.dtype
    nat.check(nat.lib().msocr_upsample2x_bilinear(x.data_ptr(), N, H, W, C, _pixel_dense_ld(x), _dt(x), out.data_ptr(),
                                                  _pixel_dense_ld(out), _stream()), "upsample2x")
    return out


def east_head(h1, w9, b9, score=None, geo=None):
    _need_cuda(h1, w9, b9)
    N, H, W, C = h1.shape
    assert C == 32 and w9.shape == (9, 32) and w9.dtype == torch.float32
    if score is None:
        score = torch.empty((N, H, W), dtype=torch.float32, device=h1.device)
    if geo is None:
        geo = torch.empty((N, H, W, 8), dtype=torch.float32, device=h1.device)
    nat.check(nat.lib().msocr_east_head(h1.data_ptr(), N * H * W, _pixel_dense_ld(h1), _dt(h1), w9.data_ptr(), b9.data_ptr(),
                                        score.data_ptr(), geo.data_ptr(), _stream()), "east_head")
    return score, geo


def east_decode(score, geo, thresh, scale, quant, max_cand):
    _need_cuda(score, geo)
    N, H, W = score.shape
    assert score.dtype == torch.float32 and geo.shape == (N, H, W, 8) and score.is_contiguous() and geo.is_contiguous()
    cand = torch.empty((N, max_cand, 9), dtype=torch.float32, device=score.device)
    counts = torch.empty((N,), dtype=torch.int32, device=score.device)
    nat.check(nat.lib().msocr_east_decode(score.data_ptr(), geo.data_ptr(), N, H, W, float(thresh), float(scale), int(quant),
                                          cand.data_ptr(), counts.data_ptr(), max_cand, _stream()), "east_decode")
    return cand, counts


def east_lanms(cand, counts, iou_thr, workspace=None):
    _need_cuda(cand, counts)
    N, max_cand, _ = cand.shape
    if workspace is None:
        nbytes = nat.lib().msocr_lanms_workspace_bytes(N, max_cand)
        workspace = torch.empty((nbytes,), dtype=torch.uint8, device=cand.device)
    boxes = torch.empty_like(cand)
    nbox = torch.empty((N,), dtype=torch.int32, device=cand.device)
    nat.check(nat.lib().msocr_east_lanms(cand.data_ptr(), counts.data_ptr(), N, max_cand, float(iou_thr), boxes.data_ptr(),
                                         nbox.data_ptr(), workspace.data_ptr(), _stream()), "east_lanms")
    return boxes, nbox


def east_box_tail(boxes, nbox, expand_w, expand_h, scale_x, scale_y, axis_aligned, remove_anomalies, sigma, min_count):
    _need_cuda(boxes, nbox)
    N, max_cand, _ = boxes.shape
    ws = torch.empty((nat.lib().msocr_east_box_tail_workspace_bytes(N, max_cand),), dtype=torch.uint8, device=boxes.device)
    out = torch.empty_like(boxes)
    n_out = torch.empty((N,), dtype=torch.int32, device=boxes.device)
    nat.check(nat.lib().msocr_east_box_tail(boxes.data_ptr(), nbox.data_ptr(), N, max_cand, float(expand_w), float(expand_h),
                                            float(scale_x), float(scale_y), int(bool(axis_aligned)), int(bool(remove_anomalies)),
                                            float(sigma), int(min_count), out.data_ptr(), n_out.data_ptr(), ws.data_ptr(), _stream()),
              "east_box_tail")
    return out, n_out


def reading_order_crops(boxes, nbox, page_hw, min_text_size, img_h, img_w, page_base=0, y_tol_ratio=0.6, x_gap_ratio=float("inf")):
    _need_cuda(boxes, nbox)
    N, max_cand, _ = boxes.shape
    dev = boxes.device
    ws = torch.empty((nat.lib().msocr_reading_order_workspace_bytes(N, max_cand),), dtype=torch.uint8, device=dev)
    order = torch.empty((N, max_cand), dtype=torch.int32, device=dev)
    keep = torch.empty((N, max_cand), dtype=torch.int32, device=dev)
    desc = torch.empty((N, max_cand, 8), dtype=torch.int32, device=dev)
    ncrop = torch.empty((N,), dtype=torch.int32, device=dev)
    nat.check(nat.lib().msocr_reading_order_crops(boxes.data_ptr(), nbox.data_ptr(), N, max_cand, int(page_hw[0]), int(page_hw[1]),
                                                  int(min_text_size), int(img_h), int(img_w), float(y_tol_ratio), float(x_gap_ratio),
                                                  int(page_base), order.data_ptr(), keep.data_ptr(), desc.data_ptr(), ncrop.data_ptr(),
                                                  ws.data_ptr(), _stream()), "reading_order_crops")
    return order, keep, desc, ncrop


def nchw_to_nhwc(x_f32, dtype, out=None):
    _need_cuda(x_f32)
    N, C, H, W = x_f32.shape
    assert x_f32.dtype == torch.float32 and x_f32.is_contiguous()
    if out is None:
        out = torch.empty((N, H, W, C), dtype=dtype, device=x_f32.device)
    nat.check(nat.lib().msocr_nchw_f32_to_nhwc(x_f32.data_ptr(), N, C, H, W, _dt(out), out.data_ptr(), _pixel_dense_ld(out), _stream()),
              "nchw_to_nhwc")
    return out


def nhwc_to_nchw_f32(x):
    _need_cuda(x)
    N, H, W, C = x.shape
    out = torch.empty((N, C, H, W), dtype=torch.float32, device=x.device)
    nat.check(nat.lib().msocr_nhwc_to_nchw_f32(x.data_ptr(), N, C, H, W, _pixel_dense_ld(x), _dt(x), out.data_ptr(), _stream()),
              "nhwc_to_nchw")
    return out


def se_residual(x, identity, w1, w2, out=None):
    _need_cuda(x, identity, w1, w2)
    N, H, W, C = x.shape
    assert x.is_contiguous() and identity.is_contiguous() and identity.shape == x.shape and identity.dtype == x.dtype
    assert w1.shape == (C // 16, C) and w2.shape == (C, C // 16) and w1.dtype == torch.float32
    if out is None:
        out = torch.empty_like(x)
    gate = torch.empty((N, C), dtype=torch.float32, device=x.device)
    e = _prof_begin()
    nat.check(nat.lib().msocr_se_residual(x.data_ptr(), identity.data_ptr(), N, H * W, C, _dt(x), w1.data_ptr(), w2.data_ptr(),
                                          gate.data_ptr(), out.data_ptr(), _stream()), "se_residual")
    _prof_end(e, "se_residual", 3.0 * x.element_size() * N * H * W * C, (N, H * W, C))
    return out


def mean_over_h(x):
    _need_cuda(x)
    N, H, W, C = x.shape
    assert x.is_contiguous()
    out = torch.empty((N, W, C), dtype=torch.float32, device=x.device)
    nat.check(nat.lib().msocr_mean_over_h(x.data_ptr(), N, H, W, C, _dt(x), out.data_ptr(), _stream()), "mean_over_h")
    return out


def bilstm_recurrent(xproj, whh_t, B, T, H, whh_planes=None):
    _need_cuda(xproj, whh_t)
    assert xproj.is_contiguous() and xproj.numel() == B * T * 8 * H and whh_t.shape == (2, H, H, 4) and whh_t.is_contiguous()
    out = torch.empty((B, T, 2 * H), dtype=torch.float32, device=xproj.device)
    e = _prof_begin()
    if whh_planes is not None and H == 256 and SPLIT_BF16X3 and B * T * 8 * H < 2 ** 32:
        nat.check(nat.lib().msocr_bilstm_recurrent_split(xproj.data_ptr(), whh_planes.data_ptr(), B, T, H, out.data_ptr(), _stream()),
                  "bilstm_recurrent_split")
    else:
        nat.check(nat.lib().msocr_bilstm_recurrent(xproj.data_ptr(), whh_t.data_ptr(), B, T, H, out.data_ptr(), _stream()), "bilstm_recurrent")
    _prof_end(e, "bilstm", (2.0 * T * (4.0 * H * H * 4 + B * (H + H + 4 * H) * 4 * 2), T), (B, T, H))
    return out


def crop_descriptors(boxes, page_ids, page_hw, img_h, img_w):
    import numpy as np
    H, W = page_hw
    b = np.asarray(boxes, dtype=np.int64).reshape(-1, 4)
    pg = np.asarray(page_ids, dtype=np.int64).reshape(-1)
    a_, b_ = np.maximum(0, b[:, 0]), np.maximum(0, b[:, 1])
    c_, d_ = np.minimum(W, b[:, 2]), np.minimum(H, b[:, 3])
    c_ = np.where(c_ < 0, np.maximum(W + c_, 0), c_)
    d_ = np.where(d_ < 0, np.maximum(H + d_, 0), d_)
    keep = (c_ > a_) & (d_ > b_)
    a_, b_, c_, d_, pg = a_[keep], b_[keep], c_[keep], d_[keep], pg[keep]
    h, w = d_ - b_, c_ - a_
    scale = np.minimum(img_h / np.maximum(h, 1), img_w / np.maximum(w, 1))
    nw = np.maximum(1, np.rint(w * scale).astype(np.int64))
    nh = np.maximum(1, np.rint(h * scale).astype(np.int64))
    yy = np.maximum(0, np.minimum((img_h - nh) // 2, img_h - nh))
    desc = np.stack([pg, a_, b_, c_, d_, nw, nh, yy], axis=1).astype(np.int32) if len(pg) else np.zeros((0, 8), dtype=np.int32)
    return desc, keep


def _crop_descriptors_loop(boxes, page_ids, page_hw, img_h, img_w):
    import numpy as np
    H, W = page_hw
    desc, keep = [], []
    for (x0, y0, x1, y1), pg in zip(boxes, page_ids):
        a, b = max(0, int(x0)), max(0, int(y0))
        c, d = min(W, int(x1)), min(H, int(y1))
        if c < 0:
            c = max(W + c, 0)
        if d < 0:
            d = max(H + d, 0)
        if c <= a or d <= b:
            keep.append(False)
            continue
        h, w = d - b, c - a
        scale = min(img_h / max(h, 1), img_w / max(w, 1))
        nw, nh = max(1, int(round(w * scale))), max(1, int(round(h * scale)))
        yy = max(0, min((img_h - nh) // 2, img_h - nh))
        desc.append((pg, a, b, c, d, nw, nh, yy))
        keep.append(True)
    return np.asarray(desc, dtype=np.int32).reshape(-1, 8), np.asarray(keep, dtype=bool)


def crop_resize_pad(pages_u8, desc_host, img_h, img_w, desc_dev=None):
    _need_cuda(pages_u8, desc_dev)
    N, H, W, C = pages_u8.shape
    assert C == 3 and pages_u8.dtype == torch.uint8 and pages_u8.is_contiguous()
    hp = None
    if desc_host is not None:
        desc_host = desc_host.astype("int32", copy=False)
        hp = desc_host.ctypes.data
    M = len(desc_host) if desc_host is not None else int(desc_dev.shape[0])
    if desc_dev is None:
        desc_dev = torch.from_numpy(desc_host).to(pages_u8.device)
    else:
        assert desc_dev.dtype == torch.int32 and desc_dev.is_contiguous() and desc_dev.shape == (M, 8)
        desc_dev.record_stream(torch.cuda.current_stream())
    out = torch.empty((M, img_h, img_w, 3), dtype=torch.uint8, device=pages_u8.device)
    nat.check(nat.lib().msocr_crop_resize_pad(pages_u8.data_ptr(), N, H, W, desc_dev.data_ptr(), hp, M, img_h, img_w,
                                              out.data_ptr(), _stream()), "crop_resize_pad")
    return out
```

manuscript_ocr_amd/recognizers/_trba/net.py:

```python
import ctypes

import numpy as np

import torch

from ... import _native as nat
from ... import ops
from ...detectors._east.net import BN_EPS, pack_stem_weight, stem_view, to_khwc


def _fold(sd, conv_key, bn_key):
    w = sd[conv_key + ".weight"].float()
    gamma, beta = sd[bn_key + ".weight"].float(), sd[bn_key + ".bias"].float()
    mean, var = sd[bn_key + ".running_mean"].float(), sd[bn_key + ".running_var"].float()
    s = gamma / torch.sqrt(var + BN_EPS)
    return w * s.view(-1, 1, 1, 1), beta - mean * s


def _gate_interleave(w_t, H):
    K = w_t.shape[0]
    return w_t.reshape(K, 4, H).permute(0, 2, 1).contiguous()


HOIST_CTX = True

LAYER_SPEC = (("layer1", 1, 2), ("layer2", 2, 1), ("layer3", 5, 2), ("layer4", 3, 1))


class TrbaNet:
    def __init__(self, state_dict, num_classes, hidden=256, dtype=torch.float32, device="cuda", split=None):
        check_decoder_shape(hidden, num_classes)
        self.dtype, self.device = dtype, torch.device(device)
        self.V, self.Hd = num_classes, hidden
        dev, sd = self.device, state_dict
        P = {}
        self.cpad = 4 if dtype == torch.float32 else 8
        self.cin_pad = 16 if dtype == torch.float32 else 32
        w, b = _fold(sd, "cnn.conv0.0", "cnn.conv0.1")
        P["stem"] = (pack_stem_weight(w, self.cin_pad, self.cpad).to(dtype).to(dev), b.to(dev))
        w, b = _fold(sd, "cnn.conv0.3", "cnn.conv0.4")
        P["conv0b"] = (to_khwc(w, dtype, dev, split), b.to(dev))
        for lname, blocks, stride in LAYER_SPEC:
            for i in range(blocks):
                p = f"cnn.{lname}.{i}."
                for j in (1, 2):
                    w, b = _fold(sd, p + f"conv{j}", p + f"bn{j}")
                    P[f"{lname}.{i}.conv{j}"] = (to_khwc(w, dtype, dev, split), b.to(dev))
                P[f"{lname}.{i}.se"] = (sd[p + "se.fc.0.weight"].float().contiguous().to(dev),
                                        sd[p + "se.fc.2.weight"].float().contiguous().to(dev))
                if p + "downsample.0.weight" in sd:
                    w, b = _fold(sd, p + "downsample.0", p + "downsample.1")
                    P[f"{lname}.{i}.down"] = (to_khwc(w, dtype, dev, split), b.to(dev))
        w, b = _fold(sd, "cnn.conv_out.0", "cnn.conv_out.1")
        P["out0"] = (to_khwc(w, dtype, dev, split), b.to(dev))
        w, b = _fold(sd, "cnn.conv_out.3", "cnn.conv_out.4")
        P["out1"] = (to_khwc(w, dtype, dev, split), b.to(dev))
        self.P = P
        H = hidden
        self.rnn = []
        for l in (0, 1):
            p = f"enc_rnn.{l}."
            w_ih = torch.cat([sd[p + "rnn.weight_ih_l0"], sd[p + "rnn.weight_ih_l0_reverse"]]).float()
            b = torch.cat([sd[p + "rnn.bias_ih_l0"] + sd[p + "rnn.bias_hh_l0"],
                           sd[p + "rnn.bias_ih_l0_reverse"] + sd[p + "rnn.bias_hh_l0_reverse"]]).float()
            whh_t = torch.stack([_gate_interleave(sd[p + "rnn.weight_hh_l0"].float().t(), H),
                                 _gate_interleave(sd[p + "rnn.weight_hh_l0_reverse"].float().t(), H)])
            whh_p = None
            if (ops.SPLIT_BF16X3 if split is None else split) and dtype == torch.float32 and H == 256:
                n = nat.lib().msocr_attn_pack_split_elems(4 * H)
                packed = torch.empty((2, n), dtype=torch.int16)
                wt = whh_t.contiguous()
                for d in (0, 1):
                    nat.check(nat.lib().msocr_attn_pack_split_host(wt[d].data_ptr(), 4 * H, 1, packed[d].data_ptr()), "attn_pack_split_host")
                whh_p = packed.to(dev)
            self.rnn.append({
                "w_ih": w_ih.view(8 * H, 1, 1, -1).contiguous().to(dev), "b": b.contiguous().to(dev),
                "whh_t": whh_t.contiguous().to(dev), "whh_p": whh_p,
                "lin_w": sd[p + "linear.weight"].float().view(H, 1, 1, 2 * H).contiguous().to(dev),
                "lin_b": sd[p + "linear.bias"].float().contiguous().to(dev),
            })
        self.dec = AttnDecoder(state_dict, num_classes, hidden, split, device,
                               step_split=bool((ops.SPLIT_BF16X3 if split is None else split) and dtype == torch.float32))
        self.att, self._aw, self._asw = self.dec.att, self.dec._aw, self.dec._asw

    def _se_block(self, x, lname, i, stride):
        P = self.P
        w1, b1 = P[f"{lname}.{i}.conv1"]
        w2, b2 = P[f"{lname}.{i}.conv2"]
        o = ops.conv2d(x, w1, b1, stride=(stride, stride), pad=(1, 1), relu=True)
        o = ops.conv2d(o, w2, b2, pad=(1, 1))
        key = f"{lname}.{i}.down"
        idt = ops.conv2d(x, *P[key], stride=(stride, stride)) if key in P else x
        s1, s2 = P[f"{lname}.{i}.se"]
        return ops.se_residual(o, idt, s1, s2)

    def cnn(self, canvases_u8):
        B, h, w, _ = canvases_u8.shape
        x = ops.normalize_u8(canvases_u8, 1, 1, h + 2, w + 4, 1, self.dtype, cpad=self.cpad)
        ws, bs = self.P["stem"]
        x = ops.conv2d(stem_view(x, self.cin_pad), ws, bs, (1, 1), (0, 0), True, out_hw=(h, w), alg_k=27)
        x = ops.conv2d(x, *self.P["conv0b"], pad=(1, 1), relu=True, pool2=True)
        for lname, blocks, stride in LAYER_SPEC:
            for i in range(blocks):
                x = self._se_block(x, lname, i, stride if i == 0 else 1)
        x = ops.conv2d(x, *self.P["out0"], stride=(2, 1), pad=(0, 1), relu=True)
        return ops.conv2d(x, *self.P["out1"], relu=True)

    def _gemm(self, x2d, w, b):
        return _gemm(x2d, w, b)

    def encode(self, canvases_u8):
        f = self.cnn(canvases_u8)
        B, Hf, T, C = f.shape
        seq = ops.mean_over_h(f)
        H = self.Hd
        for l in (0, 1):
            r = self.rnn[l]
            xproj = self._gemm(seq.view(B * T, -1), r["w_ih"], r["b"])
            hcat = ops.bilstm_recurrent(xproj, r["whh_t"], B, T, H, r["whh_p"])
            seq = self._gemm(hcat.view(B * T, 2 * H), r["lin_w"], r["lin_b"]).view(B, T, H)
        proj = self._gemm(seq.view(B * T, H), self.att["i2h_w"], None).view(B, T, H)
        return seq, proj

    def greedy(self, batch_H, proj_H, max_len, sos_id, eos_id, blank_id):
        return self.dec.greedy(batch_H, proj_H, max_len, sos_id, eos_id, blank_id)

    def beam(self, batch_H, proj_H, max_len, beam_size, alpha, temperature, sos_id, eos_id, blank_id, chunks=None):
        return self.dec.beam(batch_H, proj_H, max_len, beam_size, alpha, temperature, sos_id, eos_id, blank_id, chunks)

    def beam_finalize(self, ws, B, steps, beam_size, trun_dev):
        return self.dec.beam_finalize(ws, B, steps, beam_size, trun_dev)


def check_decoder_shape(hidden, num_classes):
    if hidden % 64 or not 64 <= hidden <= 512:
        raise ValueError(f"hidden_size must be a multiple of 64 between 64 and 512 for the HIP recurrent / attention kernels, got {hidden}")
    if num_classes > 512:
        raise ValueError(f"charsets above 512 tokens are not supported by the decoder kernels, got {num_classes}")


def _gemm(x2d, w, b):
    M, K = x2d.shape
    return ops.conv2d(x2d.view(1, M, 1, K), w, b).view(M, w.shape[0])


class AttnDecoder:

    def __init__(self, state_dict, num_classes, hidden=256, split=None, device="cuda", step_split=None):
        check_decoder_shape(hidden, num_classes)
        if step_split is None:
            step_split = bool(ops.SPLIT_BF16X3 if split is None else split)
        self.device = torch.device(device)
        self.V, self.Hd = num_classes, hidden
        dev, sd, H = self.device, state_dict, hidden
        a = "attn.attention_cell."
        w_ih = sd[a + "rnn.weight_ih"].float()
        self.att = {
            "i2h_w": sd[a + "i2h.weight"].float().view(H, 1, 1, H).contiguous().to(dev),
            "h2h_wt": sd[a + "h2h.weight"].float().t().contiguous().to(dev),
            "h2h_b": sd[a + "h2h.bias"].float().contiguous().to(dev),
            "score_w": sd[a + "score.weight"].float().view(H).contiguous().to(dev),
            "wih_ctx_t": _gate_interleave(w_ih[:, :H].t(), H).to(dev),
            "wih_tok": _gate_interleave(w_ih[:, H:].t(), H).to(dev),
            "whh_t": _gate_interleave(sd[a + "rnn.weight_hh"].float().t(), H).to(dev),
            "b_gates": _gate_interleave((sd[a + "rnn.bias_ih"] + sd[a + "rnn.bias_hh"]).float().view(1, 4 * H), H).view(H, 4).contiguous().to(dev),
            "gen_wt": sd["attn.generator.weight"].float().t().contiguous().to(dev),
            "gen_b": sd["attn.generator.bias"].float().contiguous().to(dev),
        }
        self.att["wih_ctx_rows"] = ops.attach_split(w_ih[:, :H].reshape(4, H, H).permute(1, 0, 2).reshape(4 * H, 1, 1, H).contiguous().to(dev),
                                                    split)
        aw = nat.AttnWeights()
        for k in ("h2h_wt", "h2h_b", "score_w", "wih_ctx_t", "wih_tok", "whh_t", "b_gates", "gen_wt", "gen_b"):
            setattr(aw, k, self.att[k].data_ptr())
        self._aw = aw
        self._asw = None
        if step_split and H == 256 and self.V <= 256:
            asw = nat.AttnSplitWeights()
            for src, dst, n, gi in (("h2h_wt", "h2h_p", H, 0), ("whh_t", "whh_p", 4 * H, 1), ("gen_wt", "gen_p", self.V, 0)):
                wt = self.att[src].cpu().contiguous()
                packed = torch.empty((nat.lib().msocr_attn_pack_split_elems(n),), dtype=torch.int16)
                nat.check(nat.lib().msocr_attn_pack_split_host(wt.data_ptr(), n, gi, packed.data_ptr()), "attn_pack_split_host")
                self.att[dst] = packed.to(dev)
                setattr(asw, dst, self.att[dst].data_ptr())
            self._asw = asw

    def _matrix_core(self, T, beam_size=None):
        if not HOIST_CTX or self.Hd != 256 or self.V > 256 or T > 48:
            return False
        return self._asw is not None if beam_size is None else beam_size <= 8

    def ctx_gates(self, batch_H):
        B, T, H = batch_H.shape
        return _gemm(batch_H.reshape(B * T, H), self.att["wih_ctx_rows"], None)

    def greedy(self, batch_H, proj_H, max_len, sos_id, eos_id, blank_id, ctx_gates=None):
        B, T, H = batch_H.shape
        steps = max_len + 1
        logits = torch.empty((B, steps, self.V), dtype=torch.float32, device=self.device)
        ids = torch.empty((B, steps), dtype=torch.int32, device=self.device)
        blank = -1 if blank_id is None else blank_id
        if self._matrix_core(T):
            ctxg = self.ctx_gates(batch_H) if ctx_gates is None else ctx_gates
            nat.check(nat.lib().msocr_attn_greedy_hoisted(batch_H.data_ptr(), proj_H.data_ptr(), ctxg.data_ptr(), ctypes.byref(self._aw),
                                                          ctypes.byref(self._asw), B, T, H, self.V, steps, sos_id, eos_id, blank,
                                                          logits.data_ptr(), ids.data_ptr(), ops._stream()), "attn_greedy_hoisted")
        else:
            nat.check(nat.lib().msocr_attn_greedy(batch_H.data_ptr(), proj_H.data_ptr(), ctypes.byref(self._aw), B, T, H, self.V, steps,
                                                  sos_id, eos_id, blank, logits.data_ptr(), ids.data_ptr(), ops._stream()), "attn_greedy")
        return logits, ids

    def beam(self, batch_H, proj_H, max_len, beam_size, alpha, temperature, sos_id, eos_id, blank_id, chunks=None, ctx_gates=None):
        B, T, H = batch_H.shape
        steps = max_len
        nbytes = nat.lib().msocr_attn_beam_workspace_bytes(B, steps, beam_size, self.V)
        ws = torch.empty((nbytes,), dtype=torch.uint8, device=self.device)
        fin = torch.empty((B,), dtype=torch.int32, device=self.device)
        lp = None
        if alpha > 0:
            key = (float(alpha), steps)
            if not hasattr(self, "_lp_cache"):
                self._lp_cache = {}
            if key not in self._lp_cache:
                self._lp_cache[key] = torch.tensor([((5.0 + (t + 1)) ** alpha) / (6.0 ** alpha) for t in range(steps)],
                                                   dtype=torch.float32).to(self.device)
                torch.cuda.synchronize()
            lp = self._lp_cache[key]
        if not 1 <= beam_size <= 16 or beam_size * H > 4096:
            raise ValueError(f"beam_size {beam_size} with hidden_size {H}: the decoder kernels take beam_size <= 16 and beam_size x hidden_size <= 4096")
        hoist = self._matrix_core(T, beam_size)
        if hoist:
            ctxg = self.ctx_gates(batch_H) if ctx_gates is None else ctx_gates
        e = ops._prof_begin()
        tail = (B, T, H, self.V, steps, beam_size, lp.data_ptr() if lp is not None else None, float(temperature), sos_id, eos_id,
                -1 if blank_id is None else blank_id, fin.data_ptr(), ws.data_ptr(),
                chunks[0].data_ptr() if chunks else None, chunks[1].data_ptr() if chunks else None,
                chunks[2].data_ptr() if chunks else None, ops._stream())
        if hoist:
            asw = ctypes.byref(self._asw) if self._asw is not None else None
            nat.check(nat.lib().msocr_attn_beam_hoisted(batch_H.data_ptr(), proj_H.data_ptr(), ctxg.data_ptr(), ctypes.byref(self._aw),
                                                        asw, *tail), "attn_beam_hoisted")
        else:
            nat.check(nat.lib().msocr_attn_beam(batch_H.data_ptr(), proj_H.data_ptr(), ctypes.byref(self._aw), *tail), "attn_beam")
        V, R = self.V, B * beam_size
        per_step = 4.0 * (2 * B * T * H + 4 * H * (H + V) + 4 * H * H + H * V + H * H + R * (4 * H + V))
        ops._prof_end(e, "attn_beam", (per_step, steps), (B, T, beam_size))
        return ws, fin, lp

    def beam_finalize(self, ws, B, steps, beam_size, trun_dev):
        logits = torch.empty((B, steps, self.V), dtype=torch.float32, device=self.device)
        ids = torch.empty((B, steps), dtype=torch.int32, device=self.device)
        nat.check(nat.lib().msocr_attn_beam_finalize(ws.data_ptr(), B, self.V, steps, beam_size, trun_dev.data_ptr(), logits.data_ptr(),
                                                     ids.data_ptr(), ops._stream()), "attn_beam_finalize")
        return logits, ids


def trba_cnn_macs(h, w):
    macs = h * w * 64 * 27 + h * w * 128 * 64 * 9
    hh, ww, cin = h // 2, w // 2, 128
    for (lname, blocks, stride), planes in zip(LAYER_SPEC, (256, 256, 512, 512)):
        for i in range(blocks):
            s = stride if i == 0 else 1
            h2, w2 = (hh + 2 - 3) // s + 1, (ww + 2 - 3) // s + 1
            macs += h2 * w2 * planes * cin * 9 + h2 * w2 * planes * planes * 9
            if s != 1 or cin != planes:
                macs += h2 * w2 * planes * cin
            macs += 2 * planes * (planes // 16)
            hh, ww, cin = h2, w2, planes
    h3, w3 = (hh - 2) // 2 + 1, (ww + 2 - 2) + 1
    macs += h3 * w3 * 512 * 512 * 4
    macs += (h3 - 1) * (w3 - 1) * 512 * 512 * 4
    return macs
```

Measured before the change: 80.63.

## Chain Winograd transforms across SE-block convs and fuse SE residual into input transform

Inside each stride-1 SE block, conv1's Winograd output transform now writes straight into conv2's Winograd input domain through a new chain-transform kernel. The conv1 activation is therefore never stored in spatial form and read back. The SE residual epilogue is also fused with the next block's Winograd input transform: an LDS-staged kernel applies the gate, adds the residual, applies ReLU, writes the output and emits the V tiles in one pass. The cost is extra kernels, large LDS footprints per channel slice, and a shared helper header. It also adds new preconditions such as power-of-two C and a fit check, with a fallback to the old path when they are not met.

Result: no change. 80.16 (median of 4 runs) (-0.6%).

```diff
diff --git a/include/msocr.h b/include/msocr.h
--- a/include/msocr.h
+++ b/include/msocr.h
@@ -44,6 +44,11 @@
 int msocr_winograd_output_transform(const msocr_conv_desc* d, int form, const void* workspace, const float* bias, const void* residual,
                                     void* out, void* stream);
 
+int msocr_wino_chain_channels(int H, int W, int C, int tiles);
+int msocr_winograd_chain_supported(const msocr_conv_desc* d1, int form1, const msocr_conv_desc* d2, int form2);
+int msocr_winograd_chain_transform(const msocr_conv_desc* d1, int form1, const void* workspace1, const float* bias,
+                                   const msocr_conv_desc* d2, int form2, void* workspace2, void* stream);
+
 int msocr_split_bf16x3_host(const float* w_host, int64_t n, uint16_t* planes_out_host);
 int msocr_split_bf16x3_ktile_host(const float* w_host, int64_t nbatch, int64_t rows, int64_t k, uint16_t* planes_out_host);
 int msocr_conv1x1_split(const msocr_conv_desc* d, const void* in, const void* weight_planes, const float* bias,
@@ -89,6 +94,8 @@
 
 int msocr_se_residual(const void* x, const void* identity, int N, int HW, int C, int dtype, const float* w1,
                       const float* w2, float* gate_ws, void* out, void* stream);
+int msocr_se_residual_winograd(const void* x, const void* identity, int N, int H, int W, int C, const float* w1, const float* w2,
+                               float* gate_ws, void* out, int form, void* V, void* stream);
 
 int msocr_mean_over_h(const void* in, int N, int H, int W, int C, int dtype, float* out, void* stream);
 
diff --git a/manuscript_ocr_amd/_native.py b/manuscript_ocr_amd/_native.py
--- a/manuscript_ocr_amd/_native.py
+++ b/manuscript_ocr_amd/_native.py
@@ -46,6 +46,9 @@
     "msocr_winograd_input_transform": (c_i32, [ctypes.POINTER(ConvDesc), c_i32, c_vp, c_vp, c_vp]),
     "msocr_winograd_gemm": (c_i32, [ctypes.POINTER(ConvDesc), c_i32, c_i32, c_vp, c_vp, c_vp]),
     "msocr_winograd_output_transform": (c_i32, [ctypes.POINTER(ConvDesc), c_i32, c_vp, c_vp, c_vp, c_vp, c_vp]),
+    "msocr_wino_chain_channels": (c_i32, [c_i32, c_i32, c_i32, c_i32]),
+    "msocr_winograd_chain_supported": (c_i32, [ctypes.POINTER(ConvDesc), c_i32, ctypes.POINTER(ConvDesc), c_i32]),
+    "msocr_winograd_chain_transform": (c_i32, [ctypes.POINTER(ConvDesc), c_i32, c_vp, c_vp, ctypes.POINTER(ConvDesc), c_i32, c_vp, c_vp]),
     "msocr_winograd_fused64_workspace_bytes": (c_i64, [ctypes.POINTER(ConvDesc)]),
     "msocr_conv3x3_winograd_fused64": (c_i32, [ctypes.POINTER(ConvDesc), c_i32, c_vp, c_vp, c_vp, c_vp, c_vp, c_vp, c_vp]),
     "msocr_winograd_fused64_gemm_output": (c_i32, [ctypes.POINTER(ConvDesc), c_i32, c_vp, c_vp, c_vp, c_vp, c_vp, c_vp]),
@@ -62,6 +65,7 @@
     "msocr_lanms_workspace_bytes": (c_i64, [c_i32, c_i32]),
     "msocr_east_lanms": (c_i32, [c_vp, c_vp, c_i32, c_i32, c_f64, c_vp, c_vp, c_vp, c_vp]),
     "msocr_se_residual": (c_i32, [c_vp, c_vp, c_i32, c_i32, c_i32, c_i32, c_vp, c_vp, c_vp, c_vp, c_vp]),
+    "msocr_se_residual_winograd": (c_i32, [c_vp, c_vp, c_i32, c_i32, c_i32, c_i32, c_vp, c_vp, c_vp, c_vp, c_i32, c_vp, c_vp]),
     "msocr_mean_over_h": (c_i32, [c_vp, c_i32, c_i32, c_i32, c_i32, c_i32, c_vp, c_vp]),
     "msocr_bilstm_recurrent": (c_i32, [c_vp, c_vp, c_i32, c_i32, c_i32, c_vp, c_vp]),
     "msocr_bilstm_recurrent_split": (c_i32, [c_vp, c_vp, c_i32, c_i32, c_i32, c_vp, c_vp]),
diff --git a/manuscript_ocr_amd/csrc/trba_kernels.hip b/manuscript_ocr_amd/csrc/trba_kernels.hip
--- a/manuscript_ocr_amd/csrc/trba_kernels.hip
+++ b/manuscript_ocr_amd/csrc/trba_kernels.hip
@@ -4,11 +4,10 @@
 
 #include "internal.h"
 #include "msocr.h"
+#include "winograd_tile.h"
 
 #define MSOCR_LAUNCH(...) do { (void)hipGetLastError(); hipLaunchKernelGGL(__VA_ARGS__); } while (0)
 #define LAUNCH_OK() (hipGetLastError() == hipSuccess ? MSOCR_OK : MSOCR_E_LAUNCH)
-
-typedef float f32x4 __attribute__((ext_vector_type(4)));
 
 __device__ __forceinline__ float bf2f(uint16_t v) { return __uint_as_float(((uint32_t)v) << 16); }
 __device__ __forceinline__ uint16_t f2bf(float f) {
@@ -53,10 +52,8 @@
 }
 
 template <typename T, int NT>
-__global__ __launch_bounds__(NT) void se_residual_kernel(const T* __restrict__ x, const T* __restrict__ idt, int HW, int C,
-                                                           const float* __restrict__ w1, const float* __restrict__ w2,
-                                                           float* __restrict__ gate_ws, T* __restrict__ out) {
-  extern __shared__ __attribute__((aligned(16))) float sm[];
+__device__ __forceinline__ void se_gate_body(const T* __restrict__ x, int HW, int C, const float* __restrict__ w1,
+                                             const float* __restrict__ w2, float* __restrict__ gate_ws, float* sm) {
   const int n = blockIdx.x, tid = threadIdx.x;
   const int C4 = C / 4, PG = NT / C4;
   float* part = sm;
@@ -108,6 +105,26 @@
     gate_ws[(long)n * C + c] = g;
   }
   __syncthreads();
+}
+
+__device__ __forceinline__ f32x4 se_scale4(f32x4 v, f32x4 g4, f32x4 r) {
+  f32x4 y;
+#pragma unroll
+  for (int e = 0; e < 4; ++e) y[e] = fmaxf(v[e] * g4[e] + r[e], 0.f);
+  return y;
+}
+
+template <typename T, int NT>
+__global__ __launch_bounds__(NT) void se_residual_kernel(const T* __restrict__ x, const T* __restrict__ idt, int HW, int C,
+                                                           const float* __restrict__ w1, const float* __restrict__ w2,
+                                                           float* __restrict__ gate_ws, T* __restrict__ out) {
+  extern __shared__ __attribute__((aligned(16))) float sm[];
+  se_gate_body<T, NT>(x, HW, C, w1, w2, gate_ws, sm);
+  const int n = blockIdx.x, tid = threadIdx.x;
+  const int C4 = C / 4, PG = NT / C4;
+  const float* gate = sm + PG * C + C + C / 16;
+  const T* xs = x + (long)n * HW * C;
+  const int cg = tid % C4, pg = tid / C4;
   const T* is = idt + (long)n * HW * C;
   T* os = out + (long)n * HW * C;
   const f32x4 g4 = *reinterpret_cast<const f32x4*>(&gate[cg * 4]);
@@ -121,21 +138,39 @@
       r[u] = ld4<T>(is + o);
     }
 #pragma unroll
-    for (int u = 0; u < 4; ++u) {
-      f32x4 y;
-#pragma unroll
-      for (int e = 0; e < 4; ++e) y[e] = fmaxf(v[u][e] * g4[e] + r[u][e], 0.f);
-      st4<T>(os + (long)(p + u * PG) * C + cg * 4, y);
-    }
+    for (int u = 0; u < 4; ++u) st4<T>(os + (long)(p + u * PG) * C + cg * 4, se_scale4(v[u], g4, r[u]));
   }
   for (; p < HW; p += PG) {
     const long o = (long)p * C + cg * 4;
-    const f32x4 v = ld4<T>(xs + o), r = ld4<T>(is + o);
-    f32x4 y;
-#pragma unroll
-    for (int e = 0; e < 4; ++e) y[e] = fmaxf(v[e] * g4[e] + r[e], 0.f);
-    st4<T>(os + o, y);
-  }
+    st4<T>(os + o, se_scale4(ld4<T>(xs + o), g4, ld4<T>(is + o)));
+  }
+}
+
+template <int NT>
+__global__ __launch_bounds__(NT) void se_gate_kernel(const float* __restrict__ x, int HW, int C, const float* __restrict__ w1,
+                                                     const float* __restrict__ w2, float* __restrict__ gate_ws) {
+  extern __shared__ __attribute__((aligned(16))) float sm[];
+  se_gate_body<float, NT>(x, HW, C, w1, w2, gate_ws, sm);
+}
+
+template <int MH, int MW>
+__global__ __launch_bounds__(256) void wino_input_kernel_se(const float* __restrict__ x, const float* __restrict__ idt, int C, WinoGeom g,
+                                                            const float* __restrict__ gate_ws, int CS, float* __restrict__ out,
+                                                            float* __restrict__ V) {
+  extern __shared__ __attribute__((aligned(16))) float map[];
+  const int nsl = C / CS;
+  const int n = blockIdx.x / nsl, c0 = (blockIdx.x - n * nsl) * CS;
+  const int q4 = CS >> 2, HW = g.H * g.W;
+  for (int it = threadIdx.x; it < HW * q4; it += 256) {
+    const int p = it / q4, cq = (it - p * q4) << 2;
+    const long o = ((long)n * HW + p) * C + c0 + cq;
+    const f32x4 g4 = *reinterpret_cast<const f32x4*>(gate_ws + (long)n * C + c0 + cq);
+    const f32x4 y = se_scale4(ld4<float>(x + o), g4, ld4<float>(idt + o));
+    st4<float>(out + o, y);
+    *reinterpret_cast<f32x4*>(map + p * CS + cq) = y;
+  }
+  __syncthreads();
+  wino_input_from_lds<MH, MW>(map, CS, n, c0, C, g, V);
 }
 
 extern "C" int msocr_se_residual(const void* x, const void* identity, int N, int HW, int C, int dtype, const float* w1, const float* w2,
@@ -151,6 +186,36 @@
   } else {
     return MSOCR_E_ARG;
   }
+  return LAUNCH_OK();
+}
+
+extern "C" int msocr_se_residual_winograd(const void* x, const void* identity, int N, int H, int W, int C, const float* w1, const float* w2,
+                                          float* gate_ws, void* out, int form, void* V, void* stream) {
+  if (!x || !identity || !w1 || !w2 || !gate_ws || !out || !V || N <= 0 || H <= 0 || W <= 0 || C < 64 || C > 1024 || (C & (C - 1)))
+    return MSOCR_E_ARG;
+  if (form < MSOCR_WINO_2X2 || form > MSOCR_WINO_4X4 || (((uintptr_t)x | (uintptr_t)identity | (uintptr_t)out | (uintptr_t)V) & 15))
+    return MSOCR_E_ARG;
+  static const int tile[3][2] = {{2, 2}, {4, 2}, {4, 4}};
+  WinoGeom g;
+  g.N = N; g.H = H; g.W = W;
+  g.TH = (H + tile[form][0] - 1) / tile[form][0]; g.TW = (W + tile[form][1] - 1) / tile[form][1];
+  g.Mt = (long)N * g.TH * g.TW;
+  const int CS = msocr_wino_chain_channels(H, W, C, g.TH * g.TW);
+  if (CS <= 0 || (long)N * (C / 4) > 0x7fffffffL) return MSOCR_E_ARG;
+  hipStream_t s = (hipStream_t)stream;
+  const int HW = H * W;
+  MSOCR_LAUNCH((se_gate_kernel<1024>), dim3(N), dim3(1024), (size_t)((1024 / (C / 4)) * C + 2 * C + C / 16) * sizeof(float), s,
+               (const float*)x, HW, C, w1, w2, gate_ws);
+  if (hipGetLastError() != hipSuccess) return MSOCR_E_LAUNCH;
+  const dim3 grid((unsigned)((long)N * (C / CS)));
+  const size_t lds = (size_t)HW * CS * sizeof(float);
+  const float* xp = (const float*)x;
+  const float* ip = (const float*)identity;
+  float* op = (float*)out;
+  float* vp = (float*)V;
+  if (form == MSOCR_WINO_2X2) MSOCR_LAUNCH((wino_input_kernel_se<2, 2>), grid, dim3(256), lds, s, xp, ip, C, g, gate_ws, CS, op, vp);
+  else if (form == MSOCR_WINO_4X2) MSOCR_LAUNCH((wino_input_kernel_se<4, 2>), grid, dim3(256), lds, s, xp, ip, C, g, gate_ws, CS, op, vp);
+  else MSOCR_LAUNCH((wino_input_kernel_se<4, 4>), grid, dim3(256), lds, s, xp, ip, C, g, gate_ws, CS, op, vp);
   return LAUNCH_OK();
 }
 
diff --git a/manuscript_ocr_amd/csrc/winograd.hip b/manuscript_ocr_amd/csrc/winograd.hip
--- a/manuscript_ocr_amd/csrc/winograd.hip
+++ b/manuscript_ocr_amd/csrc/winograd.hip
@@ -3,62 +3,12 @@
 
 #include "internal.h"
 #include "msocr.h"
+#include "winograd_tile.h"
 
 #define MSOCR_LAUNCH(...) do { (void)hipGetLastError(); hipLaunchKernelGGL(__VA_ARGS__); } while (0)
-
-typedef float f32x4 __attribute__((ext_vector_type(4)));
-
-template <int M> __device__ void wino_bt1(const f32x4 d[M + 2], f32x4 r[M + 2]);
-template <int M> __device__ void wino_at1(const f32x4 m[M + 2], f32x4 y[M]);
-
-template <> __device__ __forceinline__ void wino_bt1<2>(const f32x4 d[4], f32x4 r[4]) {
-  r[0] = d[0] - d[2];
-  r[1] = d[1] + d[2];
-  r[2] = d[2] - d[1];
-  r[3] = d[1] - d[3];
-}
-template <> __device__ __forceinline__ void wino_at1<2>(const f32x4 m[4], f32x4 y[2]) {
-  y[0] = (m[0] + m[1]) + m[2];
-  y[1] = (m[1] - m[2]) - m[3];
-}
-
-__device__ __forceinline__ void wino44_bt(const f32x4 d[6], f32x4 r[6]) {
-  constexpr float k97_36 = 97.0f / 36.0f, k4_9 = 4.0f / 9.0f, k9_4 = 2.25f, k3_2 = 1.5f, k2_3 = 2.0f / 3.0f;
-#pragma unroll
-  for (int e = 0; e < 4; ++e) {
-    r[0][e] = fmaf(-k97_36, d[2][e], d[0][e]) + d[4][e];
-    r[5][e] = fmaf(-k97_36, d[3][e], d[1][e]) + d[5][e];
-    const float e1 = fmaf(-k4_9, d[2][e], d[4][e]), o1 = fmaf(k3_2, d[3][e], -k2_3 * d[1][e]);
-    const float e2 = fmaf(-k9_4, d[2][e], d[4][e]), o2 = fmaf(k2_3, d[3][e], -k3_2 * d[1][e]);
-    r[1][e] = e1 + o1; r[2][e] = e1 - o1;
-    r[3][e] = e2 + o2; r[4][e] = e2 - o2;
-  }
-}
-__device__ __forceinline__ void wino44_at(const f32x4 m[6], f32x4 y[4]) {
-  constexpr float k3_2 = 1.5f, k2_3 = 2.0f / 3.0f, k9_4 = 2.25f, k4_9 = 4.0f / 9.0f, k27_8 = 3.375f, k8_27 = 8.0f / 27.0f;
-#pragma unroll
-  for (int e = 0; e < 4; ++e) {
-    const float p12 = m[1][e] + m[2][e], d12 = m[1][e] - m[2][e], p34 = m[3][e] + m[4][e], d34 = m[3][e] - m[4][e];
-    y[0][e] = (m[0][e] + p12) + p34;
-    y[1][e] = fmaf(k3_2, d12, k2_3 * d34);
-    y[2][e] = fmaf(k9_4, p12, k4_9 * p34);
-    y[3][e] = fmaf(k27_8, d12, k8_27 * d34) + m[5][e];
-  }
-}
-template <> __device__ __forceinline__ void wino_bt1<4>(const f32x4 d[6], f32x4 r[6]) { wino44_bt(d, r); }
-template <> __device__ __forceinline__ void wino_at1<4>(const f32x4 m[6], f32x4 y[4]) { wino44_at(m, y); }
-
-
-struct WinoGeom {
-  int N, H, W;
-  int TH, TW;
-  long Mt;
-};
 
 template <int MH, int MW>
 __device__ __forceinline__ void wino_input_body(const float* in, long sN, long sH, long sW, int C, WinoGeom g, float* V) {
-  constexpr int PH = MH + 2, PW = MW + 2;
-  constexpr bool w_first = MH == 4;
   const int cch = C >> 2;
   const long gid = (long)blockIdx.x * 256 + threadIdx.x;
   const long t = gid / cch;
@@ -70,61 +20,29 @@
   const int n = (int)(r / g.TH);
   const int h0 = MH * th - 1, w0 = MW * tw - 1;
   const float* base = in + (long)n * sN + c;
-  f32x4 q[PH][PW];
-#pragma unroll
-  for (int i = 0; i < PH; ++i) {
-    const int hi = h0 + i;
-    const bool okh = (unsigned)hi < (unsigned)g.H;
-    f32x4 d[PW];
-#pragma unroll
-    for (int j = 0; j < PW; ++j) {
-      const int wi = w0 + j;
-      const bool ok = okh && (unsigned)wi < (unsigned)g.W;
-      const f32x4 v = *reinterpret_cast<const f32x4*>(ok ? base + (long)hi * sH + (long)wi * sW : base);
-      d[j] = ok ? v : (f32x4){0.f, 0.f, 0.f, 0.f};
-    }
-    if constexpr (w_first) {
-      wino_bt1<MW>(d, q[i]);
-    } else {
-#pragma unroll
-      for (int j = 0; j < PW; ++j) q[i][j] = d[j];
-    }
-  }
   const long plane = g.Mt * (long)C;
   float* o = V + t * (long)C + c;
-  if constexpr (w_first) {
-#pragma unroll
-    for (int j = 0; j < PW; ++j) {
-      f32x4 col[PH], v[PH];
-#pragma unroll
-      for (int i = 0; i < PH; ++i) col[i] = q[i][j];
-      wino_bt1<MH>(col, v);
-#pragma unroll
-      for (int i = 0; i < PH; ++i) *reinterpret_cast<f32x4*>(o + (i * PW + j) * plane) = v[i];
-    }
-  } else {
-#pragma unroll
-    for (int i = 0; i < PH; ++i) {
-      f32x4 row[PW], v[PW];
-#pragma unroll
-      for (int j = 0; j < PW; ++j) {
-        f32x4 col[PH], hv[PH];
-#pragma unroll
-        for (int k = 0; k < PH; ++k) col[k] = q[k][j];
-        wino_bt1<MH>(col, hv);
-        row[j] = hv[i];
-      }
-      wino_bt1<MW>(row, v);
-#pragma unroll
-      for (int j = 0; j < PW; ++j) *reinterpret_cast<f32x4*>(o + (i * PW + j) * plane) = v[j];
-    }
-  }
+  const float* rows[MH + 2];
+  bool okh[MH + 2];
+#pragma unroll
+  for (int i = 0; i < MH + 2; ++i) {
+    const int hi = h0 + i;
+    okh[i] = (unsigned)hi < (unsigned)g.H;
+    rows[i] = base + (long)hi * sH;
+  }
+  wino_input_tile<MH, MW>(
+      [&](int i, int j) {
+        const int wi = w0 + j;
+        const bool ok = okh[i] && (unsigned)wi < (unsigned)g.W;
+        const f32x4 v = *reinterpret_cast<const f32x4*>(ok ? rows[i] + (long)wi * sW : base);
+        return ok ? v : (f32x4){0.f, 0.f, 0.f, 0.f};
+      },
+      [&](int p, f32x4 v) { *reinterpret_cast<f32x4*>(o + p * plane) = v; });
 }
 
 template <int MH, int MW>
 __device__ __forceinline__ void wino_output_body(const float* Mw, int Cout, WinoGeom g, const float* bias, const float* res, long res_ld,
                                                  int relu, float* out, long out_ld) {
-  constexpr int PH = MH + 2, PW = MW + 2;
   const int cch = Cout >> 2;
   const long gid = (long)blockIdx.x * 256 + threadIdx.x;
   const long t = gid / cch;
@@ -136,44 +54,14 @@
   const int n = (int)(r / g.TH);
   const long plane = g.Mt * (long)Cout;
   const float* mp = Mw + t * (long)Cout + c;
-  f32x4 mt[PH][PW];
-  if constexpr (MH == 2) {
-#pragma unroll
-    for (int i = 0; i < PH; ++i)
-#pragma unroll
-      for (int j = 0; j < PW; ++j) mt[i][j] = *reinterpret_cast<const f32x4*>(mp + (i * PW + j) * plane);
-  }
-  f32x4 s[MH][PW];
-#pragma unroll
-  for (int j = 0; j < PW; ++j) {
-    f32x4 m[PH], y[MH];
-#pragma unroll
-    for (int i = 0; i < PH; ++i) m[i] = MH == 2 ? mt[i][j] : *reinterpret_cast<const f32x4*>(mp + (i * PW + j) * plane);
-    wino_at1<MH>(m, y);
-#pragma unroll
-    for (int a = 0; a < MH; ++a) s[a][j] = y[a];
-  }
   f32x4 b = {0.f, 0.f, 0.f, 0.f};
   if (bias) b = *reinterpret_cast<const f32x4*>(bias + c);
-#pragma unroll
-  for (int a = 0; a < MH; ++a) {
-    const int ho = MH * th + a;
-    if (ho >= g.H) continue;
-    f32x4 y[MW];
-    wino_at1<MW>(s[a], y);
-#pragma unroll
-    for (int j = 0; j < MW; ++j) {
-      const int wo = MW * tw + j;
-      if (wo >= g.W) continue;
-      const long pix = ((long)n * g.H + ho) * g.W + wo;
-      f32x4 v = y[j] + b;
-      if (res) v += *reinterpret_cast<const f32x4*>(res + pix * res_ld + c);
-      if (relu) {
-        v[0] = fmaxf(v[0], 0.f); v[1] = fmaxf(v[1], 0.f); v[2] = fmaxf(v[2], 0.f); v[3] = fmaxf(v[3], 0.f);
-      }
-      *reinterpret_cast<f32x4*>(out + pix * out_ld + c) = v;
-    }
-  }
+  wino_output_tile<MH, MW>(
+      [&](int p) { return *reinterpret_cast<const f32x4*>(mp + p * plane); }, MH * th, MW * tw, g.H, g.W,
+      [&](int ho, int wo, f32x4 y) {
+        const long pix = ((long)n * g.H + ho) * g.W + wo;
+        *reinterpret_cast<f32x4*>(out + pix * out_ld + c) = wino_act(y, b, res, pix * res_ld + c, relu);
+      });
 }
 
 #define WINO_TRANSFORM_KERNELS(PREFIX, MH, MW)                                                                                    \
@@ -287,6 +175,79 @@
   rc = msocr_winograd_gemm(d, form, split, u, workspace, stream);
   if (rc != MSOCR_OK) return rc;
   return msocr_winograd_output_transform(d, form, workspace, bias, residual, out, stream);
+}
+
+template <int MH1, int MW1, int MH2, int MW2>
+__global__ __launch_bounds__(256) void wino_output_kernel_chain(const float* __restrict__ Mw, int C, WinoGeom g1, WinoGeom g2,
+                                                                const float* __restrict__ bias, int relu, int CS, float* __restrict__ V) {
+  extern __shared__ __attribute__((aligned(16))) float map[];
+  const int nsl = C / CS;
+  const int n = blockIdx.x / nsl, c0 = (blockIdx.x - n * nsl) * CS;
+  const int q4 = CS >> 2, tiles = g1.TH * g1.TW;
+  const long plane = g1.Mt * (long)C;
+  for (int it = threadIdx.x; it < tiles * q4; it += 256) {
+    const int tl = it / q4, cq = (it - tl * q4) << 2;
+    const int th = tl / g1.TW, tw = tl - th * g1.TW;
+    const float* mp = Mw + ((long)n * tiles + tl) * C + c0 + cq;
+    f32x4 b = {0.f, 0.f, 0.f, 0.f};
+    if (bias) b = *reinterpret_cast<const f32x4*>(bias + c0 + cq);
+    wino_output_tile<MH1, MW1>(
+        [&](int p) { return *reinterpret_cast<const f32x4*>(mp + p * plane); }, MH1 * th, MW1 * tw, g1.H, g1.W,
+        [&](int ho, int wo, f32x4 y) { *reinterpret_cast<f32x4*>(map + (ho * g1.W + wo) * CS + cq) = wino_act(y, b, nullptr, 0, relu); });
+  }
+  __syncthreads();
+  wino_input_from_lds<MH2, MW2>(map, CS, n, c0, C, g2, V);
+}
+
+template <int MH1, int MW1>
+static void wino_chain_launch(int form2, dim3 grid, size_t lds, hipStream_t st, const float* Mw, int C, const WinoGeom& g1,
+                              const WinoGeom& g2, const float* bias, int relu, int CS, float* V) {
+  if (form2 == MSOCR_WINO_2X2) MSOCR_LAUNCH((wino_output_kernel_chain<MH1, MW1, 2, 2>), grid, dim3(256), lds, st, Mw, C, g1, g2, bias, relu, CS, V);
+  else if (form2 == MSOCR_WINO_4X2) MSOCR_LAUNCH((wino_output_kernel_chain<MH1, MW1, 4, 2>), grid, dim3(256), lds, st, Mw, C, g1, g2, bias, relu, CS, V);
+  else MSOCR_LAUNCH((wino_output_kernel_chain<MH1, MW1, 4, 4>), grid, dim3(256), lds, st, Mw, C, g1, g2, bias, relu, CS, V);
+}
+
+extern "C" int msocr_wino_chain_channels(int H, int W, int C, int tiles) {
+  if (H <= 0 || W <= 0 || C <= 0 || C % 4 || tiles <= 0) return -1;
+  const long px = (long)H * W;
+  if (px * 4 * (long)sizeof(float) > kWinoChainLds) return -1;
+  int cs = 4;
+  while (cs * 2 <= C && C % (cs * 2) == 0 && (long)tiles * cs / 4 < 256 && px * cs * 2 * (long)sizeof(float) <= kWinoChainLds) cs *= 2;
+  return cs;
+}
+
+static int wino_chain_check(const msocr_conv_desc* d1, int form1, const msocr_conv_desc* d2, int form2, WinoGeom* g1, WinoGeom* g2) {
+  if (wino_check(d1, form1, g1) != MSOCR_OK || wino_check(d2, form2, g2) != MSOCR_OK) return -1;
+  if (d1->Cout != d2->Cin || d1->N != d2->N || d1->H != d2->H || d1->W != d2->W) return -1;
+  if (d1->flags & (MSOCR_CONV_RESIDUAL | MSOCR_CONV_POOL2)) return -1;
+  if ((long)d1->N * (d1->Cout / 4) > 0x7fffffffL) return -1;
+  return msocr_wino_chain_channels(d1->H, d1->W, d1->Cout, (int)(g1->TH * g1->TW));
+}
+
+extern "C" int msocr_winograd_chain_supported(const msocr_conv_desc* d1, int form1, const msocr_conv_desc* d2, int form2) {
+  WinoGeom g1, g2;
+  return wino_chain_check(d1, form1, d2, form2, &g1, &g2) > 0 ? 1 : 0;
+}
+
+extern "C" int msocr_winograd_chain_transform(const msocr_conv_desc* d1, int form1, const void* workspace1, const float* bias,
+                                              const msocr_conv_desc* d2, int form2, void* workspace2, void* stream) {
+  WinoGeom g1, g2;
+  const int CS = wino_chain_check(d1, form1, d2, form2, &g1, &g2);
+  if (CS <= 0 || !workspace1 || !workspace2 || (((uintptr_t)workspace1 | (uintptr_t)workspace2) & 15)) return MSOCR_E_ARG;
+  if (bias && ((uintptr_t)bias & 15)) return MSOCR_E_ARG;
+  const float* Mw = (const float*)workspace1 + wino_points(form1) * g1.Mt * (long)d1->Cin;
+  float* V = (float*)workspace2;
+  const uintptr_t m0 = (uintptr_t)Mw, m1 = m0 + wino_points(form1) * g1.Mt * (uintptr_t)d1->Cout * sizeof(float);
+  const uintptr_t v0 = (uintptr_t)V, v1 = v0 + wino_points(form2) * g2.Mt * (uintptr_t)d2->Cin * sizeof(float);
+  if (v0 < m1 && m0 < v1) return MSOCR_E_ARG;
+  const dim3 grid((unsigned)((long)d1->N * (d1->Cout / CS)));
+  const size_t lds = (size_t)d1->H * d1->W * CS * sizeof(float);
+  const int relu = (d1->flags & MSOCR_CONV_RELU) ? 1 : 0;
+  hipStream_t st = (hipStream_t)stream;
+  if (form1 == MSOCR_WINO_2X2) wino_chain_launch<2, 2>(form2, grid, lds, st, Mw, d1->Cout, g1, g2, bias, relu, CS, V);
+  else if (form1 == MSOCR_WINO_4X2) wino_chain_launch<4, 2>(form2, grid, lds, st, Mw, d1->Cout, g1, g2, bias, relu, CS, V);
+  else wino_chain_launch<4, 4>(form2, grid, lds, st, Mw, d1->Cout, g1, g2, bias, relu, CS, V);
+  return hipGetLastError() == hipSuccess ? MSOCR_OK : MSOCR_E_LAUNCH;
 }
 
 typedef unsigned int u32x4w __attribute__((ext_vector_type(4)));
diff --git a/manuscript_ocr_amd/csrc/winograd_tile.h b/manuscript_ocr_amd/csrc/winograd_tile.h
--- /dev/null
+++ b/manuscript_ocr_amd/csrc/winograd_tile.h
@@ -0,0 +1,166 @@
+#ifndef MSOCR_WINOGRAD_TILE_H
+#define MSOCR_WINOGRAD_TILE_H
+#include <hip/hip_runtime.h>
+
+typedef float f32x4 __attribute__((ext_vector_type(4)));
+
+template <int M> __device__ void wino_bt1(const f32x4 d[M + 2], f32x4 r[M + 2]);
+template <int M> __device__ void wino_at1(const f32x4 m[M + 2], f32x4 y[M]);
+
+template <> __device__ __forceinline__ void wino_bt1<2>(const f32x4 d[4], f32x4 r[4]) {
+  r[0] = d[0] - d[2];
+  r[1] = d[1] + d[2];
+  r[2] = d[2] - d[1];
+  r[3] = d[1] - d[3];
+}
+template <> __device__ __forceinline__ void wino_at1<2>(const f32x4 m[4], f32x4 y[2]) {
+  y[0] = (m[0] + m[1]) + m[2];
+  y[1] = (m[1] - m[2]) - m[3];
+}
+
+__device__ __forceinline__ void wino44_bt(const f32x4 d[6], f32x4 r[6]) {
+  constexpr float k97_36 = 97.0f / 36.0f, k4_9 = 4.0f / 9.0f, k9_4 = 2.25f, k3_2 = 1.5f, k2_3 = 2.0f / 3.0f;
+#pragma unroll
+  for (int e = 0; e < 4; ++e) {
+    r[0][e] = fmaf(-k97_36, d[2][e], d[0][e]) + d[4][e];
+    r[5][e] = fmaf(-k97_36, d[3][e], d[1][e]) + d[5][e];
+    const float e1 = fmaf(-k4_9, d[2][e], d[4][e]), o1 = fmaf(k3_2, d[3][e], -k2_3 * d[1][e]);
+    const float e2 = fmaf(-k9_4, d[2][e], d[4][e]), o2 = fmaf(k2_3, d[3][e], -k3_2 * d[1][e]);
+    r[1][e] = e1 + o1; r[2][e] = e1 - o1;
+    r[3][e] = e2 + o2; r[4][e] = e2 - o2;
+  }
+}
+__device__ __forceinline__ void wino44_at(const f32x4 m[6], f32x4 y[4]) {
+  constexpr float k3_2 = 1.5f, k2_3 = 2.0f / 3.0f, k9_4 = 2.25f, k4_9 = 4.0f / 9.0f, k27_8 = 3.375f, k8_27 = 8.0f / 27.0f;
+#pragma unroll
+  for (int e = 0; e < 4; ++e) {
+    const float p12 = m[1][e] + m[2][e], d12 = m[1][e] - m[2][e], p34 = m[3][e] + m[4][e], d34 = m[3][e] - m[4][e];
+    y[0][e] = (m[0][e] + p12) + p34;
+    y[1][e] = fmaf(k3_2, d12, k2_3 * d34);
+    y[2][e] = fmaf(k9_4, p12, k4_9 * p34);
+    y[3][e] = fmaf(k27_8, d12, k8_27 * d34) + m[5][e];
+  }
+}
+template <> __device__ __forceinline__ void wino_bt1<4>(const f32x4 d[6], f32x4 r[6]) { wino44_bt(d, r); }
+template <> __device__ __forceinline__ void wino_at1<4>(const f32x4 m[6], f32x4 y[4]) { wino44_at(m, y); }
+
+
+constexpr long kWinoChainLds = 64 * 1024;
+
+struct WinoGeom {
+  int N, H, W;
+  int TH, TW;
+  long Mt;
+};
+
+template <int MH, int MW, class Ld, class St>
+__device__ __forceinline__ void wino_input_tile(Ld ld, St st) {
+  constexpr int PH = MH + 2, PW = MW + 2;
+  constexpr bool w_first = MH == 4;
+  f32x4 q[PH][PW];
+#pragma unroll
+  for (int i = 0; i < PH; ++i) {
+    f32x4 d[PW];
+#pragma unroll
+    for (int j = 0; j < PW; ++j) d[j] = ld(i, j);
+    if constexpr (w_first) {
+      wino_bt1<MW>(d, q[i]);
+    } else {
+#pragma unroll
+      for (int j = 0; j < PW; ++j) q[i][j] = d[j];
+    }
+  }
+  if constexpr (w_first) {
+#pragma unroll
+    for (int j = 0; j < PW; ++j) {
+      f32x4 col[PH], v[PH];
+#pragma unroll
+      for (int i = 0; i < PH; ++i) col[i] = q[i][j];
+      wino_bt1<MH>(col, v);
+#pragma unroll
+      for (int i = 0; i < PH; ++i) st(i * PW + j, v[i]);
+    }
+  } else {
+#pragma unroll
+    for (int i = 0; i < PH; ++i) {
+      f32x4 row[PW], v[PW];
+#pragma unroll
+      for (int j = 0; j < PW; ++j) {
+        f32x4 col[PH], hv[PH];
+#pragma unroll
+        for (int k = 0; k < PH; ++k) col[k] = q[k][j];
+        wino_bt1<MH>(col, hv);
+        row[j] = hv[i];
+      }
+      wino_bt1<MW>(row, v);
+#pragma unroll
+      for (int j = 0; j < PW; ++j) st(i * PW + j, v[j]);
+    }
+  }
+}
+
+template <int MH, int MW, class Ld, class Emit>
+__device__ __forceinline__ void wino_output_tile(Ld ld, int ho0, int wo0, int H, int W, Emit emit) {
+  constexpr int PH = MH + 2, PW = MW + 2;
+  f32x4 mt[PH][PW];
+  if constexpr (MH == 2) {
+#pragma unroll
+    for (int i = 0; i < PH; ++i)
+#pragma unroll
+      for (int j = 0; j < PW; ++j) mt[i][j] = ld(i * PW + j);
+  }
+  f32x4 s[MH][PW];
+#pragma unroll
+  for (int j = 0; j < PW; ++j) {
+    f32x4 m[PH], y[MH];
+#pragma unroll
+    for (int i = 0; i < PH; ++i) m[i] = MH == 2 ? mt[i][j] : ld(i * PW + j);
+    wino_at1<MH>(m, y);
+#pragma unroll
+    for (int a = 0; a < MH; ++a) s[a][j] = y[a];
+  }
+#pragma unroll
+  for (int a = 0; a < MH; ++a) {
+    const int ho = ho0 + a;
+    if (ho >= H) continue;
+    f32x4 y[MW];
+    wino_at1<MW>(s[a], y);
+#pragma unroll
+    for (int j = 0; j < MW; ++j) {
+      const int wo = wo0 + j;
+      if (wo >= W) continue;
+      emit(ho, wo, y[j]);
+    }
+  }
+}
+
+__device__ __forceinline__ f32x4 wino_act(f32x4 y, f32x4 b, const float* res, long roff, int relu) {
+  f32x4 v = y + b;
+  if (res) v += *reinterpret_cast<const f32x4*>(res + roff);
+  if (relu) {
+    v[0] = fmaxf(v[0], 0.f); v[1] = fmaxf(v[1], 0.f); v[2] = fmaxf(v[2], 0.f); v[3] = fmaxf(v[3], 0.f);
+  }
+  return v;
+}
+
+template <int MH, int MW>
+__device__ __forceinline__ void wino_input_from_lds(const float* map, int CS, int n, int c0, int C, WinoGeom g, float* V) {
+  const int q4 = CS >> 2, tiles = g.TH * g.TW;
+  const long plane = g.Mt * (long)C;
+  for (int it = threadIdx.x; it < tiles * q4; it += 256) {
+    const int tl = it / q4, cq = (it - tl * q4) << 2;
+    const int th = tl / g.TW, tw = tl - th * g.TW;
+    const int h0 = MH * th - 1, w0 = MW * tw - 1;
+    float* o = V + ((long)n * tiles + tl) * C + c0 + cq;
+    wino_input_tile<MH, MW>(
+        [&](int i, int j) {
+          const int hi = h0 + i, wi = w0 + j;
+          const bool ok = (unsigned)hi < (unsigned)g.H && (unsigned)wi < (unsigned)g.W;
+          const f32x4 v = *reinterpret_cast<const f32x4*>(map + (ok ? (hi * g.W + wi) * CS + cq : cq));
+          return ok ? v : (f32x4){0.f, 0.f, 0.f, 0.f};
+        },
+        [&](int p, f32x4 v) { *reinterpret_cast<f32x4*>(o + p * plane) = v; });
+  }
+}
+
+#endif
diff --git a/manuscript_ocr_amd/ops.py b/manuscript_ocr_amd/ops.py
--- a/manuscript_ocr_amd/ops.py
+++ b/manuscript_ocr_amd/ops.py
@@ -162,6 +162,19 @@
         if WINOGRAD_SQUARE and square and Cin >= WINOGRAD_SQUARE_MIN_CIN:
             w._msocr_wino44_split = split_planes_ktile(_wino_weights(wh, nat.WINO_4X4), 36, Cout).to(w.device)
     return w
+
+
+def _wino_route(H, W, w):
+    form, u, split = nat.WINO_2X2, w._msocr_wino, False
+    if WINOGRAD_TALL and _tall_pays(H) and getattr(w, "_msocr_wino42", None) is not None:
+        form, u = nat.WINO_4X2, w._msocr_wino42
+        up = getattr(w, "_msocr_wino42_split", None)
+        if up is not None and SPLIT_BF16X3:
+            u, split = up, True
+        up44 = getattr(w, "_msocr_wino44_split", None)
+        if up44 is not None and SPLIT_BF16X3 and WINOGRAD_SQUARE and _square_pays(W):
+            form, u, split = nat.WINO_4X4, up44, True
+    return form, u, split
 
 
 def _winograd(d, x, w, u, form, split, bias, residual, out, alg, fused=False, pool2=False):
@@ -254,15 +267,7 @@
         u = w._msocr_wino42_fused if up is None else up
         _winograd(d, x, w, u, nat.WINO_4X2, up is not None, bias, residual, out, alg, fused=True, pool2=pool2)
     elif use_wino:
-        form, split = nat.WINO_2X2, False
-        if WINOGRAD_TALL and _tall_pays(H) and getattr(w, "_msocr_wino42", None) is not None:
-            form, u = nat.WINO_4X2, w._msocr_wino42
-            up = getattr(w, "_msocr_wino42_split", None)
-            if up is not None and SPLIT_BF16X3:
-                u, split = up, True
-            up44 = getattr(w, "_msocr_wino44_split", None)
-            if up44 is not None and SPLIT_BF16X3 and WINOGRAD_SQUARE and _square_pays(W):
-                form, u, split = nat.WINO_4X4, up44, True
+        form, u, split = _wino_route(H, W, w)
         _winograd(d, x, w, u, form, split, bias, residual, out, alg)
     else:
         wp = getattr(w, "_msocr_split", None)
@@ -283,6 +288,106 @@
         io = x.element_size() * (N * H * W * Cin + N * Ho * Wo * Cout * (2 if residual is not None else 1) + Cout * KH * KW * Cin)
         _prof_end(e, "conv_gemm", (alg, 2.0 * N * Ho * Wo * Cout * KH * KW * Cin, io),
                   (N * Ho * Wo, Cout, KH * KW * Cin, "direct_split" if split else "direct"))
+    return out
+
+
+class WinoPlan:
+    def __init__(self, N, H, W, w, bias, relu, form, u, split):
+        Cout, _, _, Cin = w.shape
+        d = nat.ConvDesc()
+        d.dtype, d.N, d.H, d.W, d.Cin = nat.F32, N, H, W, Cin
+        d.in_sN, d.in_sH, d.in_sW = H * W * Cin, W * Cin, Cin
+        d.KH, d.KW, d.stride_h, d.stride_w, d.pad_h, d.pad_w = 3, 3, 1, 1, 1, 1
+        d.Ho, d.Wo, d.Cout, d.out_ld = H, W, Cout, Cout
+        d.flags = nat.CONV_RELU if relu else 0
+        self.d, self.w, self.bias, self.form, self.u, self.split = d, w, bias, form, u, split
+        self.N, self.H, self.W, self.Cin, self.Cout = N, H, W, Cin, Cout
+        self.nbytes = nat.lib().msocr_winograd_workspace_bytes(ctypes.byref(d), form)
+        _, npts, (mh, mw) = WINO_FORMS[form]
+        self.npts, self.mt = npts, N * -(-H // mh) * -(-W // mw)
+
+    def _tag(self):
+        stem = WINO_FORMS[self.form][0]
+        return stem + ("_split" if self.split else "")
+
+
+def wino_plan(N, H, W, w, bias, relu=False):
+    if w.dtype != torch.float32 or tuple(w.shape[1:3]) != (3, 3) or getattr(w, "_msocr_wino", None) is None:
+        return None
+    if getattr(w, "_msocr_wino42_fused", None) is not None:
+        return None
+    form, u, split = _wino_route(H, W, w)
+    p = WinoPlan(N, H, W, w, bias, relu, form, u, split)
+    return p if 0 < p.nbytes <= WINO_WS_LIMIT else None
+
+
+def wino_chain_supported(p1, p2):
+    L = nat.lib()
+    return (p1.Cout == p2.Cin and (p1.N, p1.H, p1.W) == (p2.N, p2.H, p2.W)
+            and p2.npts * p2.mt * p2.Cin <= p1.npts * p1.mt * p1.Cin
+            and L.msocr_winograd_chain_supported(ctypes.byref(p1.d), p1.form, ctypes.byref(p2.d), p2.form) == 1)
+
+
+def chain_workspace(p1, p2, device):
+    return _wino_workspace(max(p1.nbytes, p2.nbytes), device)
+
+
+def wino_input(p, x, ws):
+    _need_cuda(x)
+    assert x.is_contiguous() and tuple(x.shape) == (p.N, p.H, p.W, p.Cin) and x.dtype == torch.float32
+    e = _prof_begin()
+    nat.check(nat.lib().msocr_winograd_input_transform(ctypes.byref(p.d), p.form, x.data_ptr(), ws.data_ptr(), _stream()), "winograd_input_transform")
+    _prof_end(e, "wino_in", 4.0 * (p.N * p.H * p.W * p.Cin + p.npts * p.mt * p.Cin), (p.mt, p.Cin))
+
+
+def wino_gemm(p, ws):
+    e = _prof_begin()
+    nat.check(nat.lib().msocr_winograd_gemm(ctypes.byref(p.d), p.form, int(p.split), p.u.data_ptr(), ws.data_ptr(), _stream()),
+              f"winograd_gemm {p._tag()}")
+    px = p.N * p.H * p.W
+    alg = 2.0 * px * p.Cout * 9 * p.Cin
+    _prof_end(e, "conv_gemm", (alg, 2.0 * p.npts * p.mt * p.Cin * p.Cout, 4 * (px * p.Cin + px * p.Cout + p.Cout * 9 * p.Cin)),
+              (px, p.Cout, 9 * p.Cin, p._tag()))
+
+
+def wino_chain(p1, p2, ws):
+    e = _prof_begin()
+    bp = p1.bias.data_ptr() if p1.bias is not None else None
+    nat.check(nat.lib().msocr_winograd_chain_transform(ctypes.byref(p1.d), p1.form, ws.data_ptr(), bp, ctypes.byref(p2.d), p2.form,
+                                                       ws.data_ptr(), _stream()), "winograd_chain_transform")
+    _prof_end(e, "wino_out", 4.0 * (p1.npts * p1.mt * p1.Cout + p2.npts * p2.mt * p2.Cin), (p1.mt, p1.Cout))
+
+
+def wino_output(p, ws, out=None):
+    if out is None:
+        out = torch.empty((p.N, p.H, p.W, p.Cout), dtype=torch.float32, device=ws.device)
+    e = _prof_begin()
+    bp = p.bias.data_ptr() if p.bias is not None else None
+    nat.check(nat.lib().msocr_winograd_output_transform(ctypes.byref(p.d), p.form, ws.data_ptr(), bp, None, out.data_ptr(), _stream()),
+              "winograd_output_transform")
+    _prof_end(e, "wino_out", 4.0 * (p.npts * p.mt * p.Cout + p.N * p.H * p.W * p.Cout), (p.mt, p.Cout))
+    return out
+
+
+def se_winograd_supported(x, p):
+    N, H, W, C = x.shape
+    _, _, (mh, mw) = WINO_FORMS[p.form]
+    return (x.dtype == torch.float32 and (N, H, W, C) == (p.N, p.H, p.W, p.Cin) and 64 <= C <= 1024 and C & (C - 1) == 0
+            and nat.lib().msocr_wino_chain_channels(H, W, C, -(-H // mh) * -(-W // mw)) > 0)
+
+
+def se_residual_winograd(x, identity, w1, w2, p, ws, out=None):
+    _need_cuda(x, identity, w1, w2)
+    N, H, W, C = x.shape
+    assert x.is_contiguous() and identity.is_contiguous() and identity.shape == x.shape and identity.dtype == x.dtype
+    assert w1.shape == (C // 16, C) and w2.shape == (C, C // 16) and w1.dtype == torch.float32
+    if out is None:
+        out = torch.empty_like(x)
+    gate = torch.empty((N, C), dtype=torch.float32, device=x.device)
+    e = _prof_begin()
+    nat.check(nat.lib().msocr_se_residual_winograd(x.data_ptr(), identity.data_ptr(), N, H, W, C, w1.data_ptr(), w2.data_ptr(),
+                                                   gate.data_ptr(), out.data_ptr(), p.form, ws.data_ptr(), _stream()), "se_residual_winograd")
+    _prof_end(e, "se_residual", 4.0 * (4 * N * H * W * C + p.npts * p.mt * C), (N, H * W, C))
     return out
 
 
diff --git a/manuscript_ocr_amd/recognizers/_trba/net.py b/manuscript_ocr_amd/recognizers/_trba/net.py
--- a/manuscript_ocr_amd/recognizers/_trba/net.py
+++ b/manuscript_ocr_amd/recognizers/_trba/net.py
@@ -26,11 +26,14 @@
 
 LAYER_SPEC = (("layer1", 1, 2), ("layer2", 2, 1), ("layer3", 5, 2), ("layer4", 3, 1))
 
+WINO_CHAIN = True
+
 
 class TrbaNet:
     def __init__(self, state_dict, num_classes, hidden=256, dtype=torch.float32, device="cuda", split=None):
         check_decoder_shape(hidden, num_classes)
         self.dtype, self.device = dtype, torch.device(device)
+        self.exact = split is False
         self.V, self.Hd = num_classes, hidden
         dev, sd = self.device, state_dict
         P = {}
@@ -83,16 +86,43 @@
                                step_split=bool((ops.SPLIT_BF16X3 if split is None else split) and dtype == torch.float32))
         self.att, self._aw, self._asw = self.dec.att, self.dec._aw, self.dec._asw
 
-    def _se_block(self, x, lname, i, stride):
+    def _chain_plans(self, N, H, W, lname, i, stride):
+        if not WINO_CHAIN or self.exact or self.dtype != torch.float32 or stride != 1:
+            return None
+        w1, b1 = self.P[f"{lname}.{i}.conv1"]
+        w2, b2 = self.P[f"{lname}.{i}.conv2"]
+        p1 = ops.wino_plan(N, H, W, w1, b1, relu=True)
+        p2 = ops.wino_plan(N, H, W, w2, b2) if p1 is not None else None
+        return (p1, p2) if p2 is not None and ops.wino_chain_supported(p1, p2) else None
+
+    def _se_block(self, x, lname, i, stride, pend=None, nxt=None):
         P = self.P
         w1, b1 = P[f"{lname}.{i}.conv1"]
         w2, b2 = P[f"{lname}.{i}.conv2"]
-        o = ops.conv2d(x, w1, b1, stride=(stride, stride), pad=(1, 1), relu=True)
-        o = ops.conv2d(o, w2, b2, pad=(1, 1))
+        N, H, W, _ = x.shape
+        plans = pend[0] if pend is not None else self._chain_plans(N, H, W, lname, i, stride)
+        if plans is not None:
+            p1, p2 = plans
+            if pend is not None:
+                ws = pend[1]
+            else:
+                ws = ops.chain_workspace(p1, p2, x.device)
+                ops.wino_input(p1, x, ws)
+            ops.wino_gemm(p1, ws)
+            ops.wino_chain(p1, p2, ws)
+            ops.wino_gemm(p2, ws)
+            o = ops.wino_output(p2, ws)
+        else:
+            o = ops.conv2d(x, w1, b1, stride=(stride, stride), pad=(1, 1), relu=True)
+            o = ops.conv2d(o, w2, b2, pad=(1, 1))
         key = f"{lname}.{i}.down"
         idt = ops.conv2d(x, *P[key], stride=(stride, stride)) if key in P else x
         s1, s2 = P[f"{lname}.{i}.se"]
-        return ops.se_residual(o, idt, s1, s2)
+        nplans = self._chain_plans(*o.shape[:3], *nxt) if nxt is not None else None
+        if nplans is not None and ops.se_winograd_supported(o, nplans[0]):
+            ws = ops.chain_workspace(*nplans, o.device)
+            return ops.se_residual_winograd(o, idt, s1, s2, nplans[0], ws), (nplans, ws)
+        return ops.se_residual(o, idt, s1, s2), None
 
     def cnn(self, canvases_u8):
         B, h, w, _ = canvases_u8.shape
@@ -100,9 +130,10 @@
         ws, bs = self.P["stem"]
         x = ops.conv2d(stem_view(x, self.cin_pad), ws, bs, (1, 1), (0, 0), True, out_hw=(h, w), alg_k=27)
         x = ops.conv2d(x, *self.P["conv0b"], pad=(1, 1), relu=True, pool2=True)
-        for lname, blocks, stride in LAYER_SPEC:
-            for i in range(blocks):
-                x = self._se_block(x, lname, i, stride if i == 0 else 1)
+        blocks = [(lname, i, stride if i == 0 else 1) for lname, nb, stride in LAYER_SPEC for i in range(nb)]
+        pend = None
+        for k, blk in enumerate(blocks):
+            x, pend = self._se_block(x, *blk, pend=pend, nxt=blocks[k + 1] if k + 1 < len(blocks) else None)
         x = ops.conv2d(x, *self.P["out0"], stride=(2, 1), pad=(0, 1), relu=True)
         return ops.conv2d(x, *self.P["out1"], relu=True)
 
```
